# 0xSooki/stark-rs

Measured on AMD Instinct MI355X. Metric: ntt_field_elements_per_sec, higher is better.
Workload: dtype u32; 1 GPU; lde_2^22rows_x4cols_blowup8 (4 iNTT 2^22 + 4 coset NTT 2^25 per GPU per step); prime=469762049, parallelism=columns x1 (no collective)

## Files before the change

### stark_rs_amd/csrc/api.hip

```cpp
#include <condition_variable>
#include <functional>
#include <mutex>
#include <thread>

#include "hash_core.h"
#include "internal.h"
#include "lde_core.h"

const char *smi_status_string(int status) {
    switch (status) {
    case SMI_OK: return "ok";
    case SMI_ERR_NO_INVERSE: return "no inverse";
    case SMI_ERR_DIV_BY_ZERO: return "no division by zero";
    case SMI_ERR_POLY_DIV_BY_ZERO: return "No division by zero";
    case SMI_ERR_NOT_POW2: return "n must be a power of two";
    case SMI_ERR_ROOT_TOO_LARGE: return "n > 2^23 not supported by this modulus";
    case SMI_ERR_EMPTY_LEAVES: return "Cannot create tree from empty leaves";
    case SMI_ERR_LEAVES_NOT_POW2: return "Number of leaves must be power of 2";
    case SMI_ERR_INDEX_OOB: return "Index out of bounds";
    case SMI_ERR_DOMAIN_NOT_POW2: return "Domain length must be power of 2";
    case SMI_ERR_EXPANSION_NOT_POW2: return "Expansion factor must be power of 2";
    case SMI_ERR_EXPANSION_TOO_SMALL: return "Expansion factor must be at least 4";
    case SMI_ERR_CODEWORD_LEN: return "initial codeword length does not match domain length";
    case SMI_ERR_SAMPLE_ENTROPY: return "not enough entropy in indices wrt last codeword";
    case SMI_ERR_SAMPLE_TOO_MANY: return "cannot sample more indices than available in last codeword";
    case SMI_ERR_LEN_MISMATCH: return "assertion failed: domain.len() == values.len()";
    case SMI_ERR_EMPTY_DOMAIN: return "assertion failed: domain.len() > 0";
    case SMI_ERR_WRONG_FIELD: return "assertion failed: self.p == 998244353";
    case SMI_ERR_NO_ROUNDS: return "No FRI roots extracted";
    case SMI_ERR_BAD_ARG: return "bad argument";
    case SMI_ERR_NON_CANONICAL: return "field value not canonical (>= p)";
    case SMI_ERR_UNSUPPORTED_PRIME: return "unsupported modulus for this size";
    case SMI_ERR_NOT_GEOMETRIC: return "domain is not offset*omega^k";
    case SMI_ERR_COLUMNS_NOT_BOUND: return "proof has no column openings: it does not bind the column roots";
    case SMI_ERR_GRIND_EXHAUSTED: return "proof of work: no nonce below the search cap meets the difficulty";
    case SMI_ERR_HIP: return "HIP runtime error";
    case SMI_ERR_NO_DEVICE: return "no usable HIP device";
    case SMI_ERR_OOM: return "out of memory";
    case SMI_ERR_RCCL: return "RCCL / collective error";
    default: return "unknown status";
    }
}
const char *smi_version(void) { return "stark-mi 0.1 (gfx950)"; }
const char *smi_last_error(const smi_ctx *ctx) { return ctx ? ctx->err.c_str() : "null context"; }

int smi_fail(smi_ctx *ctx, int code, const char *msg) {
    if (ctx) ctx->err = msg ? msg : smi_status_string(code);
    return code;
}
int smi_hip_fail(smi_ctx *ctx, hipError_t e, const char *what) {
    if (ctx) ctx->err = std::string(what) + ": " + hipGetErrorString(e);
    (void)hipGetLastError();
    return e == hipErrorOutOfMemory ? SMI_ERR_OOM : SMI_ERR_HIP;
}

int smi_ctx_create(uint64_t p, uint64_t g, int device, smi_ctx **out) {
    if (!out) return SMI_ERR_BAD_ARG;
    *out = nullptr;
    int count = 0;
    if (hipGetDeviceCount(&count) != hipSuccess || count <= 0 || device < 0 || device >= count) return SMI_ERR_NO_DEVICE;
    smi_ctx *ctx = new smi_ctx();
    if (!field_setup(p, g, &ctx->fs)) {
        delete ctx;
        return SMI_ERR_UNSUPPORTED_PRIME;
    }
    ctx->device = device;
    int rc = SMI_OK;
    do {
        if (hipSetDevice(device) != hipSuccess) { rc = SMI_ERR_NO_DEVICE; break; }
        int cus = 0;
        if (hipDeviceGetAttribute(&cus, hipDeviceAttributeMultiprocessorCount, device) == hipSuccess && cus > 0) ctx->num_cus = cus;
        if (hipStreamCreateWithFlags(&ctx->stream, hipStreamNonBlocking) != hipSuccess) { rc = SMI_ERR_HIP; break; }
        ctx->own_stream = true;
        if (hipMalloc((void **)&ctx->d_flag, sizeof(int)) != hipSuccess) { rc = SMI_ERR_OOM; break; }
        if (hipMemsetAsync(ctx->d_flag, 0, sizeof(int), ctx->stream) != hipSuccess) { rc = SMI_ERR_HIP; break; }
        for (int dir = 0; dir < 2 && rc == SMI_OK; dir++) {
            GeomSpec sp[3];
            ntt_table_specs(ctx->fs, dir, sp);
            for (int k = 0; k < 3 && rc == SMI_OK; k++) {
                if (hipMalloc((void **)&ctx->d_tab[dir][k], ((size_t)sp[k].count * 4) << sp[k].pair) != hipSuccess) { rc = SMI_ERR_OOM; break; }
                rc = launch_geom_table(ctx, sp[k], ctx->d_tab[dir][k]);
            }
        }
        if (rc != SMI_OK) break;
        if (hipStreamSynchronize(ctx->stream) != hipSuccess) { rc = SMI_ERR_HIP; break; }
    } while (0);
    if (rc != SMI_OK) {
        smi_ctx_destroy(ctx);
        return rc;
    }
    *out = ctx;
    return SMI_OK;
}

void smi_ctx_destroy(smi_ctx *ctx) {
    if (!ctx) return;
    DeviceGuard dg__(ctx);
    (void)hipSetDevice(ctx->device);
    if (ctx->stream) (void)hipStreamSynchronize(ctx->stream);
    for (int d = 0; d < 2; d++)
        for (int k = 0; k < 3; k++) (void)hipFree(ctx->d_tab[d][k]);
    for (ScaleEntry &e : ctx->scale_cache) {
        (void)hipFree(e.lo);
        (void)hipFree(e.hi);
    }
    for (uint32_t *t : ctx->d_root_tab) (void)hipFree(t);
    (void)hipFree(ctx->scratch);
    (void)hipFree(ctx->arena);
    for (void *q : ctx->arena_overflow) (void)hipFree(q);
    for (int i = 0; i < 4; i++) (void)hipFree(ctx->tmp[i]);
    for (int i = 0; i < 2; i++) {
        if (ctx->pin[i]) (void)hipHostFree(ctx->pin[i]);
        if (ctx->pin_ev[i]) (void)hipEventDestroy(ctx->pin_ev[i]);
    }
    if (ctx->pin_out) (void)hipHostFree(ctx->pin_out);
    (void)hipFree(ctx->d_flag);
    if (ctx->own_stream && ctx->stream) (void)hipStreamDestroy(ctx->stream);
    delete ctx;
}

int smi_ctx_set_stream(smi_ctx *ctx, void *hip_stream) {
    if (!ctx) return SMI_ERR_BAD_ARG;
    DeviceGuard dg__(ctx);
    HIP_TRY(ctx, hipStreamSynchronize(ctx->stream));
    if (ctx->own_stream) (void)hipStreamDestroy(ctx->stream);
    ctx->stream = (hipStream_t)hip_stream;
    ctx->own_stream = false;
    return SMI_OK;
}
int smi_ctx_sync(smi_ctx *ctx) {
    if (!ctx) return SMI_ERR_BAD_ARG;
    DeviceGuard dg__(ctx);
    HIP_TRY(ctx, hipStreamSynchronize(ctx->stream));
    return SMI_OK;
}
int smi_ctx_profile(smi_ctx *ctx, int enable) {
    if (!ctx) return SMI_ERR_BAD_ARG;
    DeviceGuard dg__(ctx);
    ctx->prof_on = enable != 0;
    return SMI_OK;
}
int smi_ctx_profile_only(smi_ctx *ctx, const char *name_part) {
    if (!ctx) return SMI_ERR_BAD_ARG;
    if (name_part && strlen(name_part) >= sizeof ctx->prof_only) return smi_fail(ctx, SMI_ERR_BAD_ARG, "profile filter too long");
    memset(ctx->prof_only, 0, sizeof ctx->prof_only);
    if (name_part) memcpy(ctx->prof_only, name_part, strlen(name_part));
    return SMI_OK;
}
int smi_ctx_lde_two_pass(smi_ctx *ctx, int enable) {
    if (!ctx) return SMI_ERR_BAD_ARG;
    ctx->lde_two_pass = enable != 0;
    return SMI_OK;
}
int smi_ctx_copy_probe(smi_ctx *ctx, int enable) {
    if (!ctx) return SMI_ERR_BAD_ARG;
    DeviceGuard dg__(ctx);
    ctx->copy_probe = enable != 0;
    return SMI_OK;
}
int smi_ctx_profile_read(smi_ctx *ctx, smi_kernel_time *out, size_t cap, size_t *n) {
    if (!ctx || !n || (cap && !out)) return SMI_ERR_BAD_ARG;
    DeviceGuard dg__(ctx);
    HIP_TRY(ctx, hipStreamSynchronize(ctx->stream));
    size_t cnt = 0;
    for (ProfRec &r : ctx->prof) {
        float ms = 0.f;
        (void)hipEventElapsedTime(&ms, r.e0, r.e1);
        (void)hipEventDestroy(r.e0);
        (void)hipEventDestroy(r.e1);
        size_t k = 0;
        for (; k < cnt; k++)
            if (!strncmp(out[k].name, r.name, sizeof out[k].name - 1)) break;
        if (k == cnt) {
            if (cnt == cap) continue;
            memset(&out[k], 0, sizeof out[k]);
            strncpy(out[k].name, r.name, sizeof out[k].name - 1);
            cnt++;
        }
        out[k].launches++;
        out[k].total_ms += ms;
        out[k].alg_bytes += r.bytes;
        out[k].alg_mixes += r.mixes;
    }
    ctx->prof.clear();
    *n = cnt;
    return SMI_OK;
}
uint64_t smi_ctx_modulus(const smi_ctx *ctx) { return ctx ? ctx->fs.F.p : 0; }
uint32_t smi_ctx_two_adicity(const smi_ctx *ctx) { return ctx ? ctx->fs.K : 0; }

int ctx_pin_out(smi_ctx *ctx, size_t bytes, uint8_t **out) {
    if (bytes > ctx->pin_out_bytes) {
        HIP_TRY(ctx, hipStreamSynchronize(ctx->stream));
        if (ctx->pin_out) (void)hipHostFree(ctx->pin_out);
        ctx->pin_out = nullptr;
        ctx->pin_out_bytes = 0;
        const size_t want = bytes < ((size_t)2 << 20) ? ((size_t)2 << 20) : bytes + bytes / 4;
        if (hipHostMalloc(&ctx->pin_out, want, hipHostMallocDefault) != hipSuccess) {
            ctx->pin_out = nullptr;
            return smi_fail(ctx, SMI_ERR_OOM, "hipHostMalloc (result buffer)");
        }
        ctx->pin_out_bytes = want;
    }
    *out = (uint8_t *)ctx->pin_out;
    return SMI_OK;
}
int ctx_tmp(smi_ctx *ctx, int slot, size_t bytes, void **out) {
    if (bytes > ctx->tmp_bytes[slot]) {
        HIP_TRY(ctx, hipStreamSynchronize(ctx->stream));
        (void)hipFree(ctx->tmp[slot]);
        ctx->tmp[slot] = nullptr;
        ctx->tmp_bytes[slot] = 0;
        const size_t want = bytes + bytes / 4 + 256;
        if (hipMalloc(&ctx->tmp[slot], want) != hipSuccess) return smi_fail(ctx, SMI_ERR_OOM, "hipMalloc staging buffer");
        ctx->tmp_bytes[slot] = want;
    }
    *out = ctx->tmp[slot];
    return SMI_OK;
}
int arena_reset(smi_ctx *ctx) {
    if (!ctx->arena_overflow.empty() || ctx->arena_want > ctx->arena_size) {
        HIP_TRY(ctx, hipStreamSynchronize(ctx->stream));
        for (void *q : ctx->arena_overflow) (void)hipFree(q);
        ctx->arena_overflow.clear();
        if (ctx->arena_want > ctx->arena_size) {
            (void)hipFree(ctx->arena);
            ctx->arena = nullptr;
            ctx->arena_size = 0;
            const size_t want = ctx->arena_want + ctx->arena_want / 16 + (1u << 20);
            if (hipMalloc((void **)&ctx->arena, want) == hipSuccess) ctx->arena_size = want;
            else (void)hipGetLastError();
        }
    }
    ctx->arena_used = 0;
    ctx->arena_want = 0;
    return SMI_OK;
}
void *arena_alloc(smi_ctx *ctx, size_t bytes) {
    bytes = (bytes + 255) & ~(size_t)255;
    ctx->arena_want += bytes;
    if (ctx->arena_used + bytes <= ctx->arena_size) {
        void *q = ctx->arena + ctx->arena_used;
        ctx->arena_used += bytes;
        return q;
    }
    void *q = nullptr;
    if (hipMalloc(&q, bytes ? bytes : 256) != hipSuccess) {
        (void)hipGetLastError();
        return nullptr;
    }
    ctx->arena_overflow.push_back(q);
    return q;
}
int ctx_scratch(smi_ctx *ctx, size_t elems, uint32_t **out) {
    if (elems > ctx->scratch_elems) {
        HIP_TRY(ctx, hipStreamSynchronize(ctx->stream));
        (void)hipFree(ctx->scratch);
        ctx->scratch = nullptr;
        ctx->scratch_elems = 0;
        if (hipMalloc((void **)&ctx->scratch, elems * 4) != hipSuccess) return smi_fail(ctx, SMI_ERR_OOM, "hipMalloc NTT scratch");
        ctx->scratch_elems = elems;
    }
    *out = ctx->scratch;
    return SMI_OK;
}
NttTables ctx_tables(const smi_ctx *ctx, int inverse) {
    const int d = inverse ? 1 : 0;
    return NttTables{(const Tw2 *)ctx->d_tab[d][0], ctx->d_tab[d][1], ctx->d_tab[d][2], ctx->fs.K, ntt_table_h(ctx->fs.K)};
}
int ctx_root_table(smi_ctx *ctx, uint32_t log_m, const Tw2 **out) {
    if (log_m > 17 || log_m > ctx->fs.K) return smi_fail(ctx, SMI_ERR_BAD_ARG, "root table too large");
    if (!ctx->d_root_tab[log_m]) {
        const Fp &F = ctx->fs.F;
        const uint32_t w = h_root(ctx, log_m);
        const GeomSpec sp{F.r1, (uint32_t)(((uint64_t)w << 32) % F.p), 1, 1u << log_m, 1};
        uint32_t *d = nullptr;
        if (hipMalloc((void **)&d, ((size_t)8) << log_m) != hipSuccess) return smi_fail(ctx, SMI_ERR_OOM, "hipMalloc root table");
        const int rc = launch_geom_table(ctx, sp, d);
        if (rc != SMI_OK) {
            (void)hipFree(d);
            return rc;
        }
        ctx->d_root_tab[log_m] = d;
    }
    *out = (const Tw2 *)ctx->d_root_tab[log_m];
    return SMI_OK;
}
int ctx_scale_reserve(smi_ctx *ctx, size_t n) {
    if (ctx->scale_cache.size() + n < SMI_SCALE_CACHE_MAX) return SMI_OK;
    auto pinned = [&](const ScaleEntry &e) { return ctx->scale_depth > 0 && e.epoch == ctx->scale_epoch; };
    size_t want = ctx->scale_cache.size() / 2 > n ? ctx->scale_cache.size() / 2 : ctx->scale_cache.size();
    bool any = false;
    for (const ScaleEntry &e : ctx->scale_cache) any |= !pinned(e);
    if (!any) return SMI_OK;
    HIP_TRY(ctx, hipStreamSynchronize(ctx->stream));
    std::vector<ScaleEntry> keep;
    keep.reserve(ctx->scale_cache.size());
    for (const ScaleEntry &e : ctx->scale_cache) {
        if (want && !pinned(e)) {
            (void)hipFree(e.lo);
            (void)hipFree(e.hi);
            want--;
        } else {
            keep.push_back(e);
        }
    }
    ctx->scale_cache.swap(keep);
    return SMI_OK;
}
int ctx_scale_tables(smi_ctx *ctx, uint32_t c_plain, uint32_t q_plain, uint32_t L, ScaleTables *out) {
    for (ScaleEntry &e : ctx->scale_cache)
        if (e.c == c_plain && e.q == q_plain && e.L == L) {
            e.epoch = ctx->scale_epoch;
            *out = ScaleTables{e.lo, e.hi, scale_table_h(L)};
            return SMI_OK;
        }
    SMI_TRY(ctx_scale_reserve(ctx, 1));
    GeomSpec sp[2];
    scale_table_specs(ctx->fs.F, c_plain, q_plain, L, sp);
    ScaleEntry e{c_plain, q_plain, L, nullptr, nullptr, ctx->scale_epoch};
    if (hipMalloc((void **)&e.lo, (size_t)sp[0].count * 4) != hipSuccess) return smi_fail(ctx, SMI_ERR_OOM, "hipMalloc scale table");
    if (hipMalloc((void **)&e.hi, (size_t)sp[1].count * 4) != hipSuccess) {
        (void)hipFree(e.lo);
        return smi_fail(ctx, SMI_ERR_OOM, "hipMalloc scale table");
    }
    int rc = launch_geom_table(ctx, sp[0], e.lo);
    if (rc == SMI_OK) rc = launch_geom_table(ctx, sp[1], e.hi);
    if (rc != SMI_OK) {
        (void)hipFree(e.lo);
        (void)hipFree(e.hi);
        return rc;
    }
    ctx->scale_cache.push_back(e);
    *out = ScaleTables{e.lo, e.hi, scale_table_h(L)};
    return SMI_OK;
}
int check_flag(smi_ctx *ctx) {
    int flag = 0;
    HIP_TRY(ctx, hipMemcpyAsync(&flag, ctx->d_flag, sizeof(int), hipMemcpyDeviceToHost, ctx->stream));
    HIP_TRY(ctx, hipStreamSynchronize(ctx->stream));
    if (flag) {
        HIP_TRY(ctx, hipMemsetAsync(ctx->d_flag, 0, sizeof(int), ctx->stream));
        return smi_fail(ctx, SMI_ERR_NON_CANONICAL, "input field value >= p");
    }
    return SMI_OK;
}

static constexpr size_t SMI_PIN_CHUNK = (size_t)8 << 20;
static constexpr size_t SMI_PIN_MIN = (size_t)1 << 20;

static int ctx_pinned(smi_ctx *ctx) {
    for (int i = 0; i < 2; i++) {
        if (!ctx->pin[i] && hipHostMalloc(&ctx->pin[i], SMI_PIN_CHUNK * 4, hipHostMallocDefault) != hipSuccess) {
            ctx->pin[i] = nullptr;
            return smi_fail(ctx, SMI_ERR_OOM, "hipHostMalloc");
        }
        if (!ctx->pin_ev[i]) HIP_TRY(ctx, hipEventCreateWithFlags(&ctx->pin_ev[i], hipEventDisableTiming));
    }
    return SMI_OK;
}
namespace {
class HostPool {
    std::vector<std::thread> th_;
    std::mutex m_, run_m_;
    std::condition_variable work_, done_;
    std::function<void(size_t, size_t)> fn_;
    size_t n_ = 0, per_ = 0;
    unsigned gen_ = 0, pending_ = 0;
    bool stop_ = false;

    void worker(unsigned i) {
        unsigned seen = 0;
        for (;;) {
            std::unique_lock<std::mutex> lk(m_);
            work_.wait(lk, [&] { return stop_ || gen_ != seen; });
            if (stop_) return;
            seen = gen_;
            const size_t lo = (size_t)i * per_, hi = lo + per_ < n_ ? lo + per_ : n_;
            lk.unlock();
            if (lo < hi) fn_(lo, hi);
            lk.lock();
            if (--pending_ == 0) done_.notify_one();
        }
    }

public:
    explicit HostPool(unsigned t) {
        for (unsigned i = 1; i < t; i++) th_.emplace_back([this, i] { worker(i); });
    }
    ~HostPool() {
        {
            std::lock_guard<std::mutex> lk(m_);
            stop_ = true;
        }
        work_.notify_all();
        for (std::thread &x : th_) x.join();
    }
    unsigned size() const { return (unsigned)th_.size() + 1; }
    void run(size_t n, std::function<void(size_t, size_t)> fn) {
        std::lock_guard<std::mutex> serial(run_m_);
        const unsigned t = size();
        const size_t per = (n + t - 1) / t;
        {
            std::lock_guard<std::mutex> lk(m_);
            fn_ = fn;
            n_ = n;
            per_ = per;
            pending_ = t - 1;
            gen_++;
        }
        work_.notify_all();
        fn(0, per < n ? per : n);
        std::unique_lock<std::mutex> lk(m_);
        done_.wait(lk, [&] { return pending_ == 0; });
    }
};
}

template <class Fn> static void host_parallel(size_t n, Fn fn) {
    if (n < ((size_t)1 << 18)) {
        fn(0, n);
        return;
    }
    static HostPool pool([] {
        const char *e = getenv("SMI_HOST_THREADS");
        const int v = e ? atoi(e) : 0;
        unsigned hw = std::thread::hardware_concurrency();
        hw = hw < 1 ? 1 : hw;
        const unsigned cap = (unsigned)(v >= 1 && v <= 64 ? v : 8);
        return hw < cap ? hw : cap;
    }());
    pool.run(n, fn);
}

int dev_u32_to_host(smi_ctx *ctx, const uint32_t *d_in, size_t n, uint64_t *host) {
    if (!n) return SMI_OK;
    if (n < SMI_PIN_MIN) {
        void *stage;
        SMI_TRY(ctx_tmp(ctx, 0, n * 8, &stage));
        SMI_TRY(launch_widen(ctx, d_in, (uint64_t *)stage, n));
        HIP_TRY(ctx, hipMemcpyAsync(host, stage, n * 8, hipMemcpyDeviceToHost, ctx->stream));
        HIP_TRY(ctx, hipStreamSynchronize(ctx->stream));
        return SMI_OK;
    }
    SMI_TRY(ctx_pinned(ctx));
    const size_t nch = (n + SMI_PIN_CHUNK - 1) / SMI_PIN_CHUNK;
    for (size_t c = 0; c <= nch; c++) {
        if (c < nch) {
            const size_t off = c * SMI_PIN_CHUNK, cnt = n - off < SMI_PIN_CHUNK ? n - off : SMI_PIN_CHUNK;
            HIP_TRY(ctx, hipMemcpyAsync(ctx->pin[c & 1], d_in + off, cnt * 4, hipMemcpyDeviceToHost, ctx->stream));
            HIP_TRY(ctx, hipEventRecord(ctx->pin_ev[c & 1], ctx->stream));
        }
        if (c > 0) {
            const size_t off = (c - 1) * SMI_PIN_CHUNK, cnt = n - off < SMI_PIN_CHUNK ? n - off : SMI_PIN_CHUNK;
            HIP_TRY(ctx, hipEventSynchronize(ctx->pin_ev[(c - 1) & 1]));
            const uint32_t *src = (const uint32_t *)ctx->pin[(c - 1) & 1];
            uint64_t *dst = host + off;
            host_parallel(cnt, [=](size_t lo, size_t hi) {
                for (size_t i = lo; i < hi; i++) dst[i] = src[i];
            });
        }
    }
    return SMI_OK;
}

int host_to_dev_u32(smi_ctx *ctx, const uint64_t *host, size_t n, uint32_t *d_out, int reduce) {
    if (!n) return SMI_OK;
    if (n < SMI_PIN_MIN) {
        void *stage;
        SMI_TRY(ctx_tmp(ctx, 0, n * 8, &stage));
        HIP_TRY(ctx, hipMemcpyAsync(stage, host, n * 8, hipMemcpyHostToDevice, ctx->stream));
        SMI_TRY(launch_narrow(ctx, (const uint64_t *)stage, d_out, n, reduce));
        return check_flag(ctx);
    }
    SMI_TRY(ctx_pinned(ctx));
    const uint64_t p = ctx->fs.F.p;
    const size_t nch = (n + SMI_PIN_CHUNK - 1) / SMI_PIN_CHUNK;
    std::vector<int> bad(nch, 0);
    for (size_t c = 0; c < nch; c++) {
        const size_t off = c * SMI_PIN_CHUNK, cnt = n - off < SMI_PIN_CHUNK ? n - off : SMI_PIN_CHUNK;
        if (c >= 2) HIP_TRY(ctx, hipEventSynchronize(ctx->pin_ev[c & 1]));
        uint32_t *dst = (uint32_t *)ctx->pin[c & 1];
        const uint64_t *src = host + off;
        int *flag = &bad[c];
        host_parallel(cnt, [=](size_t lo, size_t hi) {
            uint64_t over = 0;
            if (reduce) {
                for (size_t i = lo; i < hi; i++) dst[i] = (uint32_t)(src[i] % p);
            } else {
                for (size_t i = lo; i < hi; i++) {
                    over |= (uint64_t)(src[i] >= p);
                    dst[i] = (uint32_t)src[i];
                }
            }
            if (over) __atomic_store_n(flag, 1, __ATOMIC_RELAXED);
        });
        HIP_TRY(ctx, hipMemcpyAsync(d_out + off, dst, cnt * 4, hipMemcpyHostToDevice, ctx->stream));
        HIP_TRY(ctx, hipEventRecord(ctx->pin_ev[c & 1], ctx->stream));
    }
    HIP_TRY(ctx, hipStreamSynchronize(ctx->stream));
    for (size_t c = 0; c < nch; c++)
        if (bad[c]) return smi_fail(ctx, SMI_ERR_NON_CANONICAL, "input field value >= p");
    return SMI_OK;
}


int smi_prim_nth_root(const smi_ctx *ctx, uint64_t n, uint64_t *out) {
    if (!ctx || !out) return SMI_ERR_BAD_ARG;
    if (!is_pow2(n)) return SMI_ERR_NOT_POW2;
    const uint32_t p = ctx->fs.F.p;
    if (ilog2(n) > ctx->fs.K) return p == 998244353u ? SMI_ERR_ROOT_TOO_LARGE : SMI_ERR_UNSUPPORTED_PRIME;
    *out = host_powmod(ctx->fs.g, (p - 1) / n, p);
    return SMI_OK;
}
int smi_ff_inv(const smi_ctx *ctx, uint64_t x, uint64_t *out) {
    if (!ctx || !out) return SMI_ERR_BAD_ARG;
    const uint32_t p = ctx->fs.F.p;
    if (x % p == 0) return SMI_ERR_NO_INVERSE;
    *out = h_inv(ctx, (uint32_t)(x % p));
    return SMI_OK;
}
int smi_ff_exp(const smi_ctx *ctx, uint64_t base, uint64_t e, uint64_t *out) {
    if (!ctx || !out) return SMI_ERR_BAD_ARG;
    *out = h_pow(ctx, (uint32_t)(base % ctx->fs.F.p), e);
    return SMI_OK;
}
int smi_ff_mul(const smi_ctx *ctx, uint64_t a, uint64_t b, uint64_t *out) {
    if (!ctx || !out) return SMI_ERR_BAD_ARG;
    const uint32_t p = ctx->fs.F.p;
    *out = h_mul(ctx, (uint32_t)(a % p), (uint32_t)(b % p));
    return SMI_OK;
}
int smi_domain_is_geometric(const smi_ctx *ctx, const uint64_t *domain, size_t n, uint64_t *offset) {
    if (!ctx || !domain || !n) return SMI_ERR_BAD_ARG;
    if (!is_pow2(n) || ilog2(n) > ctx->fs.K) return SMI_ERR_NOT_GEOMETRIC;
    const uint32_t p = ctx->fs.F.p, w = h_root(ctx, ilog2(n));
    if (domain[0] == 0 || domain[0] >= p) return SMI_ERR_NOT_GEOMETRIC;
    uint32_t x = (uint32_t)domain[0];
    for (size_t k = 1; k < n; k++) {
        x = host_mulmod(x, w, p);
        if (domain[k] != x) return SMI_ERR_NOT_GEOMETRIC;
    }
    if (offset) *offset = domain[0];
    return SMI_OK;
}

int smi_dev_alloc(smi_ctx *ctx, size_t bytes, void **d_ptr) {
    if (!ctx || !d_ptr) return SMI_ERR_BAD_ARG;
    DeviceGuard dg__(ctx);
    if (hipMalloc(d_ptr, bytes ? bytes : 1) != hipSuccess) return smi_fail(ctx, SMI_ERR_OOM, "hipMalloc");
    return SMI_OK;
}
int smi_dev_free(smi_ctx *ctx, void *d_ptr) {
    if (!ctx) return SMI_ERR_BAD_ARG;
    DeviceGuard dg__(ctx);
    HIP_TRY(ctx, hipStreamSynchronize(ctx->stream));
    HIP_TRY(ctx, hipFree(d_ptr));
    return SMI_OK;
}
int smi_dev_upload_u64(smi_ctx *ctx, const uint64_t *host, size_t n, uint32_t *d_out, int reduce) {
    if (!ctx || (!host && n) || (!d_out && n)) return SMI_ERR_BAD_ARG;
    DeviceGuard dg__(ctx);
    return host_to_dev_u32(ctx, host, n, d_out, reduce);
}
int smi_dev_download_u64(smi_ctx *ctx, const uint32_t *d_in, size_t n, uint64_t *host) {
    if (!ctx || (!host && n) || (!d_in && n)) return SMI_ERR_BAD_ARG;
    DeviceGuard dg__(ctx);
    return dev_u32_to_host(ctx, d_in, n, host);
}

int smi_dev_ntt(smi_ctx *ctx, const uint32_t *d_in, uint32_t *d_out, uint32_t log_n, size_t n_in, uint32_t batch,
// ... 437 lines not shown
```

### stark_rs_amd/csrc/emu.cpp

```cpp
#include <array>
#include <vector>

#include "ntt_driver.h"
#include "lde_core.h"
#include "tables.h"
#include "proof_parse.h"

namespace {

std::vector<uint32_t> fill(const GeomSpec &s, const Fp &F) {
    std::vector<uint32_t> t((size_t)s.count << s.pair);
    for (uint32_t i = 0; i < s.count; i++) {
        const uint32_t v = geom_entry(s.c_m, s.q_m, i, s.stride, F);
        if (s.pair) { const Tw2 c = tw2_from_mont(v, F); t[2 * i] = c.w; t[2 * i + 1] = c.q; }
        else t[i] = v;
    }
    return t;
}

template <int LOGR, int LOGW, int KIND, int CAP> void emu_pass_cols(const PassArgs &a) {
    typedef NttPass<LOGR, LOGW, KIND, CAP> NP;
    constexpr bool LAST = KIND == PASS_LAST;
    const uint32_t NT = NP::NT;
    std::vector<uint32_t> tile(NP::R * NP::WP);
    std::vector<Tw2> tw(NP::R);
    std::vector<std::array<uint32_t, 16>> mw(NT), mq(NT), iw(NT), regs(NT);
    const bool twin = KIND == PASS_MID && (a.flags & NTT_TW_IN);
    auto r16 = [](std::array<uint32_t, 16> &x) -> uint32_t(&)[16] { return reinterpret_cast<uint32_t(&)[16]>(x); };
    for (uint32_t blk = 0; blk < a.n_tiles; blk++) {
        typename NP::TileId t = NP::tile_id(a, blk);
        for (uint32_t tid = 0; tid < NT; tid++) NP::load_tw(a, tw.data(), tid);
        for (uint32_t b = 0; b < a.batch; b++) {
            if (b % NP::COLS_PER_WG == 0)
                for (uint32_t tid = 0; tid < NT; tid++) {
                    NP::out_mul(a, t, tid, r16(mw[tid]), r16(mq[tid]));
                    if (twin) NP::in_mul(a, t, tid, r16(iw[tid]));
                }
            if (twin) {
                for (uint32_t tid = 0; tid < NT; tid++) {
                    NP::template load_regs<0, false>(a, t, b, r16(regs[tid]), tid);
                    for (int i = 0; i < 16; i++) regs[tid][i] = mont_mul(regs[tid][i], iw[tid][i], a.F);
                }
                for (uint32_t tid = 0; tid < NT; tid++) NP::template step0_regs<0>(a, r16(regs[tid]), tile.data(), tw.data(), tid);
            } else if (!LAST) {
#define ZCASE(Z)                                                                                                 \
    case Z:                                                                                                      \
        for (uint32_t tid = 0; tid < NT; tid++) NP::template load_regs<Z>(a, t, b, r16(regs[tid]), tid);         \
        for (uint32_t tid = 0; tid < NT; tid++) NP::template step0_regs<Z>(a, r16(regs[tid]), tile.data(), tw.data(), tid); \
        break;
                switch (a.zlog) { ZCASE(2) ZCASE(3) ZCASE(4) default: ZCASE(0) }
#undef ZCASE
            } else if (a.flags & NTT_LAST_DIRECT) {
                for (uint32_t tid = 0; tid < NT; tid++) NP::load_rows_direct(a, t, b, r16(regs[tid]), tid);
                for (uint32_t tid = 0; tid < NT; tid++) NP::step0_rows(a, r16(regs[tid]), tile.data(), tw.data(), tid);
            } else {
                for (uint32_t tid = 0; tid < NT; tid++) NP::load_rows(a, t, b, r16(regs[tid]), tid);
                for (uint32_t tid = 0; tid < NT; tid++) NP::rows_to_lds(r16(regs[tid]), tile.data(), tid);
                for (uint32_t tid = 0; tid < NT; tid++) NP::step0_lds(a, tile.data(), tw.data(), tid);
            }
            for (uint32_t tid = 0; tid < NT; tid++) NP::step_mid(a, tile.data(), tw.data(), tid);
            for (uint32_t tid = 0; tid < NT; tid++) NP::last_step_store_mul(a, t, b, tile.data(), tw.data(), tid, r16(mw[tid]), r16(mq[tid]));
        }
    }
}

int g_share_cols = 1;

template <int LOGR, int LOGW, int KIND, int CAP> void emu_pass(const PassArgs &a, uint32_t batch) {
    typedef NttPass<LOGR, LOGW, KIND, CAP> NP;
    constexpr bool LAST = KIND == PASS_LAST;
    if (g_share_cols && NP::share_cols(a, g_share_cols == 2 ? 0u : (uint32_t)NP::COLS_MIN_WGS)) return emu_pass_cols<LOGR, LOGW, KIND, CAP>(a);
    std::vector<uint32_t> tile(NP::R * NP::WP);
    std::vector<Tw2> tw(NP::R);
    for (uint32_t b = 0; b < batch; b++)
        for (uint32_t blk = 0; blk < a.n_tiles; blk++) {
            typename NP::TileId t = NP::tile_id(a, blk);
            const uint32_t NT = NP::NT;
            for (uint32_t tid = 0; tid < NT; tid++) NP::load_tw(a, tw.data(), tid);
            if (!LAST) {
                std::vector<std::array<uint32_t, 16>> regs(NT);
#define ZCASE(Z)                                                                                                           \
    case Z:                                                                                                                \
        for (uint32_t tid = 0; tid < NT; tid++) NP::template load_regs<Z>(a, t, b, reinterpret_cast<uint32_t(&)[16]>(regs[tid]), tid); \
        for (uint32_t tid = 0; tid < NT; tid++) NP::template step0_regs<Z>(a, reinterpret_cast<uint32_t(&)[16]>(regs[tid]), tile.data(), tw.data(), tid); \
        break;
                switch (a.zlog) { ZCASE(0) ZCASE(1) ZCASE(2) ZCASE(3) ZCASE(4) }
#undef ZCASE
            } else if (a.flags & NTT_LAST_DIRECT) {
                std::vector<std::array<uint32_t, 16>> regs(NT);
                for (uint32_t tid = 0; tid < NT; tid++) NP::load_rows_direct(a, t, b, reinterpret_cast<uint32_t(&)[16]>(regs[tid]), tid);
                for (uint32_t tid = 0; tid < NT; tid++) NP::step0_rows(a, reinterpret_cast<uint32_t(&)[16]>(regs[tid]), tile.data(), tw.data(), tid);
            } else {
                for (uint32_t tid = 0; tid < NT; tid++) {
                    uint32_t v[16];
                    NP::load_rows(a, t, b, v, tid);
                    NP::rows_to_lds(v, tile.data(), tid);
                }
                for (uint32_t tid = 0; tid < NT; tid++) NP::step0_lds(a, tile.data(), tw.data(), tid);
            }
            for (uint32_t tid = 0; tid < NT; tid++) NP::step_mid(a, tile.data(), tw.data(), tid);
            for (uint32_t tid = 0; tid < NT; tid++) NP::last_step_store(a, t, b, tile.data(), tw.data(), tid);
        }
}

struct EmuLauncher {
    void small(const SmallArgs &a, uint32_t batch) {
        std::vector<uint32_t> buf((1u << a.L) + ((1u << a.L) >> 6) + 1);
        std::vector<Tw2> twm(((1u << a.L) >> 1) + 1);
        for (uint32_t tid = 0; tid < SMI_NTT_THREADS; tid++) NttSmall::load_tw(a, twm.data(), tid);
        for (uint32_t b = 0; b < batch; b++) {
            for (uint32_t tid = 0; tid < SMI_NTT_THREADS; tid++) NttSmall::load(a, b, buf.data(), tid);
            uint32_t s = 0;
            for (; s + 2 <= a.L; s += 2)
                for (uint32_t tid = 0; tid < SMI_NTT_THREADS; tid++) NttSmall::stage4(a, s, buf.data(), twm.data(), tid);
            if (s < a.L)
                for (uint32_t tid = 0; tid < SMI_NTT_THREADS; tid++) NttSmall::stage(a, s, buf.data(), twm.data(), tid);
            for (uint32_t tid = 0; tid < SMI_NTT_THREADS; tid++) NttSmall::store(a, b, buf.data(), tid);
        }
    }
    void pass(int logr, int logw, bool last, const PassArgs &a, uint32_t batch) {
#define X(LR, LW)                                           \
    if (logr == LR && logw == LW) {                         \
        const bool wide = a.F.p < (1u << 29);               \
        const int kind = last ? PASS_LAST : (a.flags & NTT_FIRST) ? PASS_FIRST : PASS_MID;   \
        if (wide && kind == PASS_FIRST) emu_pass<LR, LW, PASS_FIRST, 8>(a, batch);   \
        else if (wide && kind == PASS_MID) emu_pass<LR, LW, PASS_MID, 8>(a, batch);  \
        else if (wide) emu_pass<LR, LW, PASS_LAST, 8>(a, batch);                     \
        else if (kind == PASS_FIRST) emu_pass<LR, LW, PASS_FIRST, 4>(a, batch);      \
        else if (kind == PASS_MID) emu_pass<LR, LW, PASS_MID, 4>(a, batch);          \
        else emu_pass<LR, LW, PASS_LAST, 4>(a, batch);                               \
        return;                                             \
    }
        SMI_NTT_SHAPES(X)
#undef X
    }
};

}

static bool g_emu_last_direct = true;
extern "C" void emu_set_last_direct(int on) { g_emu_last_direct = on != 0; }
static int g_emu_defer_tw = 2;
extern "C" void emu_set_defer_tw(int mode) { g_emu_defer_tw = mode; }
extern "C" void emu_set_share_cols(int mode) { g_share_cols = mode; }
extern "C" int emu_ntt(uint64_t p, uint64_t g, const uint32_t *in, uint32_t *out, uint32_t L, uint32_t n_in,
                       uint32_t batch, uint64_t in_stride, uint64_t out_stride, int inverse, uint64_t offset,
                       uint64_t post_scale) {
    FieldSetup fs;
    if (!field_setup(p, g, &fs) || L > fs.K) return -1;
    const Fp &F = fs.F;
    GeomSpec sp[3];
    ntt_table_specs(fs, inverse, sp);
    std::vector<uint32_t> tw10 = fill(sp[0], F), lo = fill(sp[1], F), hi = fill(sp[2], F);
    NttRequest rq;
    memset(&rq, 0, sizeof rq);
    rq.T = NttTables{(const Tw2 *)tw10.data(), lo.data(), hi.data(), fs.K, ntt_table_h(fs.K)};
    std::vector<uint32_t> slo, shi;
    const uint32_t pp = F.p;
    if (!inverse) {
        rq.pre_scale = offset % pp != 1;
        if (rq.pre_scale) {
            GeomSpec s2[2];
            rq.q_plain = (uint32_t)(offset % pp);
            scale_table_specs(F, 1, (uint32_t)(offset % pp), L, s2);
            slo = fill(s2[0], F); shi = fill(s2[1], F);
        }
    } else {
        rq.post_scale = true;
        const uint32_t ninv = host_powmod((uint32_t)((1ull << L) % pp), pp - 2, pp);
        const uint32_t q = host_mulmod((uint32_t)(post_scale % pp), host_powmod((uint32_t)(offset % pp), pp - 2, pp), pp);
        GeomSpec s2[2];
        rq.q_plain = q;
        scale_table_specs(F, ninv, q, L, s2);
        slo = fill(s2[0], F); shi = fill(s2[1], F);
    }
    rq.S = ScaleTables{slo.data(), shi.data(), scale_table_h(L)};
    std::vector<uint32_t> scratch((size_t)batch << L);
    rq.in = in; rq.out = out; rq.scratch = scratch.data();
    rq.L = L; rq.n_in = n_in; rq.batch = batch; rq.in_stride = in_stride; rq.out_stride = out_stride; rq.F = F;
    rq.defer_tw = g_emu_defer_tw;
    rq.last_direct = g_emu_last_direct;
    EmuLauncher ln;
    return ntt_run(ln, rq) ? 0 : -1;
}

namespace {
struct EmuTables {
    std::vector<uint32_t> tw10, lo, hi, slo, shi;
    NttRequest rq;
};
bool emu_shard_request(uint64_t p, uint64_t g, uint32_t L, int inverse, uint64_t offset, EmuTables &t) {
    FieldSetup fs;
    if (!field_setup(p, g, &fs) || L > fs.K) return false;
    const Fp &F = fs.F;
    GeomSpec sp[3], s2[2];
    ntt_table_specs(fs, inverse, sp);
    t.tw10 = fill(sp[0], F); t.lo = fill(sp[1], F); t.hi = fill(sp[2], F);
    memset(&t.rq, 0, sizeof t.rq);
    t.rq.T = NttTables{(const Tw2 *)t.tw10.data(), t.lo.data(), t.hi.data(), fs.K, ntt_table_h(fs.K)};
    t.rq.L = L; t.rq.n_in = 1u << L; t.rq.batch = 1; t.rq.F = F;
    if (!inverse) {
        t.rq.pre_scale = offset % F.p != 1;
        t.rq.q_plain = (uint32_t)(offset % F.p);
        scale_table_specs(F, 1, t.rq.q_plain, L, s2);
    } else {
        t.rq.post_scale = true;
        t.rq.q_plain = 1;
        scale_table_specs(F, host_powmod((uint32_t)((1ull << L) % F.p), F.p - 2, F.p), 1, L, s2);
    }
    t.slo = fill(s2[0], F); t.shi = fill(s2[1], F);
    t.rq.S = ScaleTables{t.slo.data(), t.shi.data(), scale_table_h(L)};
    return true;
}
}
extern "C" int emu_ntt_shard_first(uint64_t p, uint64_t g, uint32_t *strip, uint32_t L, uint32_t log_g, uint32_t rank, int inverse, uint64_t offset) {
    EmuTables t;
    if (!emu_shard_request(p, g, L, inverse, offset, t)) return -1;
    t.rq.in = strip; t.rq.out = strip;
    EmuLauncher ln;
    return ntt_run_shard_first(ln, t.rq, log_g, rank) ? 0 : -1;
}
extern "C" int emu_ntt_shard_rest(uint64_t p, uint64_t g, uint32_t *rows, uint32_t *out, uint32_t L, uint32_t log_g, int inverse) {
    EmuTables t;
    if (!emu_shard_request(p, g, L, inverse, 1, t)) return -1;
    t.rq.scratch = rows; t.rq.out = out;
    t.rq.last_direct = g_emu_last_direct;
    EmuLauncher ln;
    return ntt_run_shard_rest(ln, t.rq, log_g) ? 0 : -1;
}

template <int LOGR, int CAP> void emu_lde_a(const LdeArgs &a) {
    typedef LdeA<LOGR, CAP> A;
    std::vector<uint32_t> tile(A::R * 4);
    std::vector<Tw2> tw(A::TWS);
    for (uint32_t b = 0; b < a.batch; b++)
        for (uint32_t blk = 0; blk < a.n_tiles; blk++) {
            const typename A::TileId t = A::tile_id(a, blk);
            std::vector<std::array<uint32_t, 16>> regs(A::NT);
            for (uint32_t tid = 0; tid < A::NT; tid++) A::load_tw(a, tw.data(), tid);
            for (uint32_t tid = 0; tid < A::NT; tid++) A::load_regs(a, t, b, reinterpret_cast<uint32_t(&)[16]>(regs[tid]), tid);
            for (uint32_t tid = 0; tid < A::NT; tid++) A::step0(a, reinterpret_cast<uint32_t(&)[16]>(regs[tid]), tile.data(), tw.data(), tid);
            for (uint32_t tid = 0; tid < A::NT; tid++) A::step_mid(a, tile.data(), tw.data(), tid);
            for (uint32_t tid = 0; tid < A::NT; tid++) A::last_step_store(a, t, b, tile.data(), tw.data(), tid);
        }
}
template <int CAP> void emu_lde_b(const LdeArgs &a) {
    typedef LdeB<CAP> B;
    std::vector<uint32_t> tile(B::R * B::WP);
    std::vector<Tw2> tw(B::R);
    for (uint32_t b = 0; b < a.batch; b++)
        for (uint32_t blk = 0; blk < a.n_tiles; blk++) {
            const typename B::TileId t = B::tile_id(a, blk);
            for (uint32_t tid = 0; tid < B::NT; tid++) B::load_tw(a, tw.data(), tid);
            for (uint32_t tid = 0; tid < B::NT; tid++) {
                uint32_t v[16];
                B::load(a, t, b, v, tid);
                B::to_lds(a, v, tile.data(), tid);
            }
            for (uint32_t tid = 0; tid < B::NT; tid++) B::step0(a, t, tile.data(), tw.data(), tid);
            for (uint32_t tid = 0; tid < B::NT; tid++) B::step_mid(a, tile.data(), tw.data(), tid);
            for (uint32_t tid = 0; tid < B::NT; tid++) B::last_step_store(a, t, b, tile.data(), tw.data(), tid);
        }
}
static int g_emu_lde_geo = -1, g_emu_lde_lay = -1;
extern "C" void emu_lde2_knobs(int geo_rq, int lay_kq) { g_emu_lde_geo = geo_rq; g_emu_lde_lay = lay_kq; }
extern "C" int emu_lde2(uint64_t p, uint64_t g, const uint32_t *coef, uint32_t *out, uint32_t L, uint32_t beta, uint32_t batch) {
    FieldSetup fs;
    if (!field_setup(p, g, &fs) || L + beta > fs.K || !lde2_supported(L, beta)) return -1;
    const Fp &F = fs.F;
    GeomSpec sp[3];
    ntt_table_specs(fs, 0, sp);
    std::vector<uint32_t> tw10 = fill(sp[0], F), lo = fill(sp[1], F), hi = fill(sp[2], F);
    std::vector<uint32_t> mid((size_t)batch << (L + beta)), coef_t((size_t)batch << L);
    const uint32_t log_m = L - SMI_LDE_LOGB + beta;
    const uint32_t wm = host_powmod(fs.wmax[0], 1ull << (fs.K - log_m), F.p);
    std::vector<uint32_t> ctab = fill(GeomSpec{F.r1, (uint32_t)(((uint64_t)wm << 32) % F.p), 1, 1u << log_m, 1}, F);
    LdeArgs a;
    memset(&a, 0, sizeof a);
    a.coef = coef; a.mid = mid.data(); a.coef_t = coef_t.data(); a.ctab = (const Tw2 *)ctab.data(); a.out = out; a.coef_stride = 1ull << L; a.out_stride = 1ull << (L + beta);
    a.F = F; a.T = NttTables{(const Tw2 *)tw10.data(), lo.data(), hi.data(), fs.K, ntt_table_h(fs.K)};
    a.L = L; a.beta = beta; a.batch = batch;
    a.geo_rq = g_emu_lde_geo >= 0 && (uint32_t)g_emu_lde_geo <= beta ? (uint32_t)g_emu_lde_geo : lde_default_geo_rq(beta);
    a.lay_kq = g_emu_lde_lay >= (int)(SMI_LDE_BLINES_LOG - a.geo_rq) && g_emu_lde_lay <= 4 ? (uint32_t)g_emu_lde_lay : SMI_LDE_BLINES_LOG - a.geo_rq;
    const bool wide = F.p < (1u << 29);
    const int logr = (int)L - SMI_LDE_LOGB;
    {
        std::vector<uint32_t> tile(LdeCoefTile::T * (LdeCoefTile::T + 1) * 4);
        for (uint32_t b = 0; b < batch; b++)
            for (uint32_t by = 0; by < (1u << logr) / LdeCoefTile::T; by++)
                for (uint32_t bx = 0; bx < 256 / LdeCoefTile::T; bx++) {
                    for (uint32_t tid = 0; tid < LdeCoefTile::NT; tid++) LdeCoefTile::load(a, bx, by, b, tile.data(), tid);
                    for (uint32_t tid = 0; tid < LdeCoefTile::NT; tid++) LdeCoefTile::store(a, bx, by, b, tile.data(), tid);
                }
    }
    a.n_tiles = 256u << beta;
#define LA(LR) if (logr == LR) { if (wide) emu_lde_a<LR, 8>(a); else emu_lde_a<LR, 4>(a); }
    LA(10) LA(11) LA(12)
#undef LA
    a.n_tiles = 1u << (L + beta - SMI_LDE_LOGB - SMI_LDE_BLINES_LOG);
    if (wide) emu_lde_b<8>(a); else emu_lde_b<4>(a);
    return 0;
}

#include "hash_core.h"
#include "merkle_plan.h"
extern "C" void emu_leaf_hash(const uint32_t *v, size_t n, uint8_t *out) {
    size_t i = 0;
    for (; i + 1 < n; i += 2) {
        uint32_t d0[8], d1[8];
        hashc::leaf_hash2(v[i], v[i + 1], d0, d1);
        memcpy(out + 32 * i, d0, 32);
        memcpy(out + 32 * (i + 1), d1, 32);
    }
    for (; i < n; i++) {
        uint32_t d[8];
        hashc::leaf_hash(v[i], d);
        memcpy(out + 32 * i, d, 32);
    }
}
extern "C" void emu_node_hash(const uint8_t *pairs, size_t n, uint8_t *out) {
    size_t i = 0;
    for (; i + 1 < n; i += 2) {
        uint32_t l0[8], r0[8], l1[8], r1[8], d0[8], d1[8];
        memcpy(l0, pairs + 64 * i, 32);
        memcpy(r0, pairs + 64 * i + 32, 32);
        memcpy(l1, pairs + 64 * (i + 1), 32);
        memcpy(r1, pairs + 64 * (i + 1) + 32, 32);
        hashc::node_hash2(l0, r0, l1, r1, d0, d1);
        memcpy(out + 32 * i, d0, 32);
        memcpy(out + 32 * (i + 1), d1, 32);
    }
    for (; i < n; i++) {
        uint32_t l[8], r[8], d[8];
        memcpy(l, pairs + 64 * i, 32);
        memcpy(r, pairs + 64 * i + 32, 32);
        hashc::node_hash(l, r, d);
        memcpy(out + 32 * i, d, 32);
    }
}
struct Q4 {
    uint32_t v[4];
    Q4() : v{0, 0, 0, 0} {}
    Q4(uint32_t x) : v{x, x, x, x} {}
    Q4(uint32_t a, uint32_t b, uint32_t c, uint32_t d) : v{a, b, c, d} {}
};
#define Q4_BIN(op)                                                 \
    inline Q4 operator op(const Q4 &a, const Q4 &b) {              \
        Q4 r;                                                      \
        for (int i = 0; i < 4; i++) r.v[i] = a.v[i] op b.v[i];     \
        return r;                                                  \
    }
Q4_BIN(+) Q4_BIN(^) Q4_BIN(&) Q4_BIN(|) Q4_BIN(*)
#undef Q4_BIN
inline Q4 operator<<(const Q4 &a, int sh) { return Q4(a.v[0] << sh, a.v[1] << sh, a.v[2] << sh, a.v[3] << sh); }
inline Q4 operator>>(const Q4 &a, int sh) { return Q4(a.v[0] >> sh, a.v[1] >> sh, a.v[2] >> sh, a.v[3] >> sh); }
namespace hashc {
#define Q4_MAP3(name)                                                          \
    inline Q4 name(const Q4 &a, const Q4 &b, const Q4 &c) {                    \
        Q4 r;                                                                  \
        for (int i = 0; i < 4; i++) r.v[i] = name(a.v[i], b.v[i], c.v[i]);     \
        return r;                                                              \
    }
Q4_MAP3(pk_mad_u16) Q4_MAP3(bfi32) Q4_MAP3(xor3) Q4_MAP3(add3)
#undef Q4_MAP3
inline Q4 dup_hi16(const Q4 &a) { return Q4(dup_hi16(a.v[0]), dup_hi16(a.v[1]), dup_hi16(a.v[2]), dup_hi16(a.v[3])); }
inline Q4 funnel16(const Q4 &hi, const Q4 &lo) {
    return Q4(funnel16(hi.v[0], lo.v[0]), funnel16(hi.v[1], lo.v[1]), funnel16(hi.v[2], lo.v[2]), funnel16(hi.v[3], lo.v[3]));
}
inline Q4 perm8(const Q4 &hi, const Q4 &lo, uint32_t sel) {
    return Q4(perm8(hi.v[0], lo.v[0], sel), perm8(hi.v[1], lo.v[1], sel), perm8(hi.v[2], lo.v[2], sel), perm8(hi.v[3], lo.v[3], sel));
}
inline void absorb32_words(Q4 P[8], const Q4 M[8]) {
    for (int i = 0; i < 4; i++) {
        uint32_t p[8], m[8];
        for (int j = 0; j < 8; j++) { p[j] = P[j].v[i]; m[j] = M[j].v[i]; }
        absorb32_words(p, m);
        for (int j = 0; j < 8; j++) P[j].v[i] = p[j];
    }
}
}
#define SMI_QUAD_EMU
namespace hashq {
#define SMI_QD inline
typedef Q4 word;
template <int P0, int P1, int P2, int P3> inline Q4 quad(const Q4 &x) { return Q4(x.v[P0], x.v[P1], x.v[P2], x.v[P3]); }
inline Q4 lane_in_quad(uint32_t) { return Q4(0, 1, 2, 3); }
inline Q4 mask_ge(const Q4 &q, uint32_t k) { return Q4(q.v[0] >= k ? ~0u : 0u, q.v[1] >= k ? ~0u : 0u, q.v[2] >= k ? ~0u : 0u, q.v[3] >= k ? ~0u : 0u); }
inline Q4 mask_eq(const Q4 &q, uint32_t k) { return Q4(q.v[0] == k ? ~0u : 0u, q.v[1] == k ? ~0u : 0u, q.v[2] == k ? ~0u : 0u, q.v[3] == k ? ~0u : 0u); }
inline Q4 sel4(const Q4 &q, const Q4 &a, const Q4 &b, const Q4 &c, const Q4 &d) {
    Q4 r;
    for (int i = 0; i < 4; i++) r.v[i] = q.v[i] == 0 ? a.v[i] : q.v[i] == 1 ? b.v[i] : q.v[i] == 2 ? c.v[i] : d.v[i];
    return r;
}
}
#include "hash_quad.h"
extern "C" void emu_node_hash_quad(const uint8_t *pairs, size_t n, uint8_t *out) {
    const hashq::Lane L = hashq::make_lane(0);
    for (size_t i = 0; i < n; i++) {
        uint32_t l[8], r[8], d[8];
        memcpy(l, pairs + 64 * i, 32);
        memcpy(r, pairs + 64 * i + 32, 32);
        Q4 ql[8], qr[8], lo, hi;
        for (int j = 0; j < 8; j++) { ql[j] = Q4(l[j]); qr[j] = Q4(r[j]); }
        hashq::node_hash(ql, qr, L, lo, hi);
        for (int q = 0; q < 4; q++) { d[q] = lo.v[q]; d[4 + q] = hi.v[q]; }
        memcpy(out + 32 * i, d, 32);
    }
}

struct H16 {
    uint32_t v[16];
    H16() { for (int i = 0; i < 16; i++) v[i] = 0; }
    H16(uint32_t x) { for (int i = 0; i < 16; i++) v[i] = x; }
};
#define H16_BIN(op)                                                \
    inline H16 operator op(const H16 &a, const H16 &b) {           \
        H16 r;                                                     \
        for (int i = 0; i < 16; i++) r.v[i] = a.v[i] op b.v[i];    \
        return r;                                                  \
    }
H16_BIN(+) H16_BIN(^) H16_BIN(&) H16_BIN(|) H16_BIN(*)
#undef H16_BIN
inline H16 operator<<(const H16 &a, int sh) { H16 r; for (int i = 0; i < 16; i++) r.v[i] = a.v[i] << sh; return r; }
inline H16 operator>>(const H16 &a, int sh) { H16 r; for (int i = 0; i < 16; i++) r.v[i] = a.v[i] >> sh; return r; }
namespace hashc {
#define H16_MAP3(name)                                                         \
    inline H16 name(const H16 &a, const H16 &b, const H16 &c) {                \
        H16 r;                                                                 \
        for (int i = 0; i < 16; i++) r.v[i] = name(a.v[i], b.v[i], c.v[i]);    \
        return r;                                                              \
    }
H16_MAP3(pk_mad_u16) H16_MAP3(bfi32) H16_MAP3(xor3)
#undef H16_MAP3
inline H16 funnel16(const H16 &hi, const H16 &lo) { H16 r; for (int i = 0; i < 16; i++) r.v[i] = funnel16(hi.v[i], lo.v[i]); return r; }
}
#define SMI_HEX_EMU
namespace hashx {
#define SMI_XD inline
typedef H16 word;
template <int N> inline H16 rot(const H16 &x) { H16 r; for (int i = 0; i < 16; i++) r.v[i] = x.v[(i - N) & 15]; return r; }
template <int N> inline H16 shr(const H16 &x) { H16 r; for (int i = 0; i < 16; i++) r.v[i] = i >= N ? x.v[i - N] : 0u; return r; }
template <int P0, int P1, int P2, int P3> inline H16 quad(const H16 &x) {
    const int P[4] = {P0, P1, P2, P3};
    H16 r;
    for (int i = 0; i < 16; i++) r.v[i] = x.v[(i & ~3) | P[i & 3]];
    return r;
}
inline H16 lane_in_row(uint32_t) { H16 r; for (int i = 0; i < 16; i++) r.v[i] = (uint32_t)i; return r; }
inline H16 mask_range(const H16 &w, uint32_t lo, uint32_t hi) { H16 r; for (int i = 0; i < 16; i++) r.v[i] = w.v[i] >= lo && w.v[i] < hi ? ~0u : 0u; return r; }
inline H16 table16(const H16 &w, const uint32_t (&t)[16]) { H16 r; for (int i = 0; i < 16; i++) r.v[i] = t[w.v[i] & 15]; return r; }
inline H16 perm8v(const H16 &hi, const H16 &lo, const H16 &sel) { H16 r; for (int i = 0; i < 16; i++) r.v[i] = hashc::perm8(hi.v[i], lo.v[i], sel.v[i]); return r; }
inline H16 lshl_or(const H16 &a, int sh, const H16 &b) { return (a << sh) | b; }
inline H16 lshl_add(const H16 &a, int sh, const H16 &b) { return (a << sh) + b; }
}
#include "hash_hex.h"
extern "C" void emu_node_hash_hex(const uint8_t *pairs, size_t n, uint8_t *out) {
    const hashx::Lane L = hashx::make_lane(0);
    for (size_t i = 0; i < n; i++) {
        uint32_t l[8], r[8];
        memcpy(l, pairs + 64 * i, 32);
        memcpy(r, pairs + 64 * i + 32, 32);
        H16 llo, lhi, rlo, rhi;
        for (int w = 0; w < 16; w++) { llo.v[w] = l[w >> 2]; lhi.v[w] = l[4 + (w >> 2)]; rlo.v[w] = r[w >> 2]; rhi.v[w] = r[4 + (w >> 2)]; }
        const H16 x = hashx::node_hash(hashx::message(llo, lhi, L), hashx::message(rlo, rhi, L), L);
        for (int w = 0; w < 16; w++) { out[32 * i + w] = (uint8_t)x.v[w]; out[32 * i + 16 + w] = (uint8_t)(x.v[w] >> 16); }
    }
}

extern "C" void emu_fs_round_hex(uint32_t *fs_words, const uint8_t *root, uint64_t *alpha) {
    const hashx::Lane L = hashx::make_lane(0);
    uint32_t r[8];
    memcpy(r, root, 32);
    H16 lo, hi, x;
    for (int w = 0; w < 16; w++) { lo.v[w] = r[w >> 2]; hi.v[w] = r[4 + (w >> 2)]; x.v[w] = fs_words[w]; }
    x = hashx::fs_absorb(x, hashx::message(lo, hi, L), L);
    for (int w = 0; w < 16; w++) fs_words[w] = x.v[w];
    const H16 y = hashx::fs_challenge(x, L);
    *alpha = 0;
    for (int k = 0; k < 8; k++) *alpha |= (uint64_t)(y.v[k] & 0xFFu) << (8 * k);
}
extern "C" void emu_fs_round(uint32_t *fs_words, const uint8_t *root, uint64_t *alpha) {
    uint32_t m[8];
    memcpy(m, root, 32);
    hashc::fs_absorb_root(fs_words, m, nullptr, alpha);
}
extern "C" void emu_fs_seed(const uint8_t *transcript, size_t len, uint32_t *fs_words, uint32_t *phase) {
    hashc::fs_seed(transcript, len, fs_words, phase);
}
extern "C" void emu_fs_absorb_root_phase(uint32_t *fs_words, uint32_t phase, const uint8_t *root, uint64_t *alpha) {
    uint32_t m[8];
    memcpy(m, root, 32);
    hashc::fs_absorb_root_phase(fs_words, m, phase, nullptr, alpha);
}
extern "C" uint64_t emu_fs_challenge_phase(const uint32_t *fs_words, uint32_t phase) { return hashc::fs_challenge_phase(fs_words, phase); }

extern "C" void emu_row_hash(const uint32_t *v, size_t n_rows, int W, uint8_t *out) {
    size_t i = 0;
    if (W >= 1 && W <= 4)
        for (; i + 1 < n_rows; i += 2) {
            uint32_t d0[8], d1[8];
            hashc::row_hash2(v + i * W, v + (i + 1) * W, W, d0, d1);
            memcpy(out + 32 * i, d0, 32);
            memcpy(out + 32 * (i + 1), d1, 32);
        }
    for (; i < n_rows; i++) {
        uint32_t d[8];
        hashc::row_hash(v + i * W, W, d);
        memcpy(out + 32 * i, d, 32);
    }
}
extern "C" void emu_row_hash_wide(const uint32_t *cols, size_t stride, size_t n, int W, uint8_t *out) {
    const uint32_t T = SMI_HASH_THREADS;
    const size_t blocks = ((n + 1) / 2 + T - 1) / T;
    for (size_t blk = 0; blk < blocks; blk++)
        for (uint32_t tid = 0; tid < T; tid++) {
            size_t i0, i1;
            bool two;
            if (!hashc::row_wide_pair(blk, tid, T, n, &i0, &i1, &two)) continue;
            uint32_t d0[8], d1[8];
            hashc::row_hash_wide2(cols, stride, i0, i1, W, d0, d1);
            memcpy(out + 32 * i0, d0, 32);
            if (two) memcpy(out + 32 * i1, d1, 32);
        }
}
extern "C" void emu_hash_bytes(const uint8_t *msg, size_t len, uint8_t *out) {
    uint32_t d[8];
    hashc::hash_bytes(msg, len, d);
    memcpy(out, d, 32);
}

#include "fri_core.h"
extern "C" int emu_fold_shard(uint64_t p, uint64_t g, const uint32_t *lo, const uint32_t *hi, uint32_t count, uint32_t i0,
                              uint32_t full_len, uint64_t alpha, uint64_t offset, uint64_t omega, uint32_t *out) {
    FieldSetup fs;
    if (!field_setup(p, g, &fs)) return -1;
    const Fp &F = fs.F;
    const uint32_t pp = F.p;
    uint32_t L = 0;
    while ((1u << L) < full_len / 2) L++;
    GeomSpec sp[2];
    scale_table_specs(F, host_powmod((uint32_t)offset, pp - 2, pp), host_powmod((uint32_t)omega, pp - 2, pp), L, sp);
    std::vector<uint32_t> slo = fill(sp[0], F), shi = fill(sp[1], F);
    const ScaleTables S{slo.data(), shi.data(), scale_table_h(L)};
    const uint32_t inv2_m = (uint32_t)(((uint64_t)host_powmod(2, pp - 2, pp) << 32) % pp);
    const uint32_t ah_m = fold_alpha_half(alpha, inv2_m, F);
    for (uint32_t i = 0; i < count; i++) out[i] = fold_element(lo[i], hi[i], i0 + i, ah_m, inv2_m, S, F);
    return 0;
}

extern "C" int emu_fold_ext(uint64_t p, uint64_t g, const uint32_t *in, uint32_t len, uint64_t stride, const uint64_t *alpha, uint64_t offset,
                            uint64_t omega, uint32_t *out, uint64_t out_stride) {
    FieldSetup fs;
    if (!field_setup(p, g, &fs) || !ext_field_ok(p, g, nullptr)) return -1;
    if (len < 2 || (len & (len - 1)) || stride < len || out_stride < len / 2 || !offset || !omega || offset >= p || omega >= p) return -1;
    const Fp &F = fs.F;
    const uint32_t pp = F.p, half = len / 2;
    uint32_t L = 0;
    while ((1u << L) < half) L++;
    GeomSpec sp[2];
    scale_table_specs(F, host_powmod((uint32_t)offset, pp - 2, pp), host_powmod((uint32_t)omega, pp - 2, pp), L, sp);
    std::vector<uint32_t> slo = fill(sp[0], F), shi = fill(sp[1], F);
    const ScaleTables S{slo.data(), shi.data(), scale_table_h(L)};
    const uint32_t inv2_m = (uint32_t)(((uint64_t)host_powmod(2, pp - 2, pp) << 32) % pp), g_m = (uint32_t)(((uint64_t)fs.g << 32) % pp);
    const ExtMul a = fold_ext_alpha(alpha, g_m, F);
    for (uint32_t i = 0; i < half; i++) {
        uint32_t l[4], h[4], o[4];
        for (int e = 0; e < 4; e++) {
            l[e] = in[e * stride + i];
            h[e] = in[e * stride + half + i];
        }
        fold_element_ext(l, h, i, a, inv2_m, S, F, o);
        for (int e = 0; e < 4; e++) out[e * out_stride + i] = o[e];
    }
    return 0;
}

extern "C" uint64_t emu_fs_rounds_ext(const uint8_t *prefix, size_t prefix_len, const uint8_t *roots, uint32_t n_roots, uint64_t *alphas) {
    uint32_t fs[16], phase = 0;
    hashc::fs_seed(prefix, prefix_len, fs, &phase);
    for (uint32_t r = 0; r < n_roots; r++) {
        uint32_t m[8];
        memcpy(m, roots + 32 * r, 32);
        if (r + 1 == n_roots) {
// ... 87 lines not shown
```

### stark_rs_amd/csrc/internal.h

```cpp
#pragma once
#include <string.h>
#include <hip/hip_runtime.h>

#include <stdlib.h>

#include <string>
#include <vector>

#include "../../include/stark_mi.h"
#include "fri_plan.h"
#include "tables.h"

struct ScaleEntry {
    uint32_t c, q, L;
    uint32_t *lo, *hi;
    uint64_t epoch;
};

struct ProfRec {
    const char *name;
    hipEvent_t e0, e1;
    double bytes;
    double mixes;
};

struct smi_ctx {
    int device = 0;
    int num_cus = 256;
    hipStream_t stream = nullptr;
    bool own_stream = false;
    FieldSetup fs;
    uint32_t *d_tab[2][3] = {{nullptr, nullptr, nullptr}, {nullptr, nullptr, nullptr}};
    std::vector<ScaleEntry> scale_cache;
    uint64_t scale_epoch = 1;
    int scale_depth = 0;
    uint32_t *d_root_tab[32] = {};
    uint32_t *scratch = nullptr;
    size_t scratch_elems = 0;
    void *tmp[4] = {nullptr, nullptr, nullptr, nullptr};
    size_t tmp_bytes[4] = {0, 0, 0, 0};
    int *d_flag = nullptr;
    void *pin[2] = {nullptr, nullptr};
    hipEvent_t pin_ev[2] = {nullptr, nullptr};
    void *pin_out = nullptr;
    size_t pin_out_bytes = 0;
    std::string err;
    bool prof_on = false;
    char prof_only[56] = {0};
    bool copy_probe = false;
    bool ntt_share_cols = !(getenv("SMI_NTT_SHARE_COLS") && atoi(getenv("SMI_NTT_SHARE_COLS")) == 0);
    bool ntt_twin_regs = !(getenv("SMI_NTT_TWIN_REGS") && atoi(getenv("SMI_NTT_TWIN_REGS")) == 0);
    bool ntt_last_direct = !(getenv("SMI_NTT_LAST_DIRECT") && atoi(getenv("SMI_NTT_LAST_DIRECT")) == 0);
    int ntt_defer_tw = getenv("SMI_NTT_DEFER_TW") ? (atoi(getenv("SMI_NTT_DEFER_TW")) != 0) : 2;
    bool lde_two_pass = getenv("SMI_LDE_TWO_PASS") && atoi(getenv("SMI_LDE_TWO_PASS"));
    std::vector<ProfRec> prof;
    uint8_t *arena = nullptr;
    size_t arena_size = 0, arena_used = 0, arena_want = 0;
    std::vector<void *> arena_overflow;
};
int arena_reset(smi_ctx *ctx);
void *arena_alloc(smi_ctx *ctx, size_t bytes);

struct ProfScope {
    smi_ctx *ctx;
    ProfRec r;
    bool on;
    ProfScope(smi_ctx *c, const char *name, double bytes, double mixes = 0.0) : ctx(c), on(c->prof_on) {
        if (on && c->prof_only[0] && !strstr(name, c->prof_only)) on = false;
        if (!on) return;
        r.name = name;
        r.bytes = bytes;
        r.mixes = mixes;
        if (hipEventCreate(&r.e0) != hipSuccess || hipEventCreate(&r.e1) != hipSuccess) { on = false; return; }
        (void)hipEventRecord(r.e0, ctx->stream);
    }
    ~ProfScope() {
        if (!on) return;
        (void)hipEventRecord(r.e1, ctx->stream);
        ctx->prof.push_back(r);
    }
};

struct DeviceGuard {
    int prev = -1;
    bool moved = false;
    explicit DeviceGuard(const smi_ctx *ctx) {
        if (!ctx) return;
        if (hipGetDevice(&prev) == hipSuccess && prev != ctx->device) moved = hipSetDevice(ctx->device) == hipSuccess;
    }
    ~DeviceGuard() {
        if (moved) (void)hipSetDevice(prev);
    }
};

struct smi_tree {
    smi_ctx *ctx;
    uint8_t *d_nodes;
    size_t n;
    bool owns;
};

int smi_hip_fail(smi_ctx *ctx, hipError_t e, const char *what);
#define HIP_TRY(ctx, call)                                             \
    do {                                                               \
        hipError_t e__ = (call);                                       \
        if (e__ != hipSuccess) return smi_hip_fail((ctx), e__, #call); \
    } while (0)
#define SMI_TRY(call)            \
    do {                         \
        int rc__ = (call);       \
        if (rc__ != SMI_OK) return rc__; \
    } while (0)

int smi_fail(smi_ctx *ctx, int code, const char *msg);
inline int smi_proof_out(smi_ctx *ctx, const std::vector<uint8_t> &bytes, uint8_t **proof, size_t *proof_len) {
    *proof = (uint8_t *)malloc(bytes.size() ? bytes.size() : 1);
    if (!*proof) return smi_fail(ctx, SMI_ERR_OOM, "malloc proof");
    memcpy(*proof, bytes.data(), bytes.size());
    *proof_len = bytes.size();
    return SMI_OK;
}

int ctx_tmp(smi_ctx *ctx, int slot, size_t bytes, void **out);
int ctx_scratch(smi_ctx *ctx, size_t elems, uint32_t **out);
int ctx_pin_out(smi_ctx *ctx, size_t bytes, uint8_t **out);
NttTables ctx_tables(const smi_ctx *ctx, int inverse);
int ctx_root_table(smi_ctx *ctx, uint32_t log_m, const Tw2 **out);
int ctx_scale_tables(smi_ctx *ctx, uint32_t c_plain, uint32_t q_plain, uint32_t L, ScaleTables *out);
#define SMI_SCALE_CACHE_MAX 96
int ctx_scale_reserve(smi_ctx *ctx, size_t n);
struct ScaleScope {
    smi_ctx *c;
    explicit ScaleScope(smi_ctx *ctx) : c(ctx) {
        if (c->scale_depth++ == 0) c->scale_epoch++;
    }
    ~ScaleScope() { c->scale_depth--; }
    ScaleScope(const ScaleScope &) = delete;
    ScaleScope &operator=(const ScaleScope &) = delete;
};

inline uint32_t h_mul(const smi_ctx *c, uint32_t a, uint32_t b) { return host_mulmod(a, b, c->fs.F.p); }
inline uint32_t h_pow(const smi_ctx *c, uint32_t a, uint64_t e) { return host_powmod(a, e, c->fs.F.p); }
inline uint32_t h_inv(const smi_ctx *c, uint32_t a) { return host_powmod(a, c->fs.F.p - 2, c->fs.F.p); }
inline uint32_t h_root(const smi_ctx *c, uint32_t log_n) {
    return host_powmod(c->fs.wmax[0], 1ull << (c->fs.K - log_n), c->fs.F.p);
}

struct FriTailRound {
    const uint32_t *cw;
    uint32_t *next;
    uint8_t *nodes;
    uint8_t *proof_slot;
    uint64_t *alpha_out;
    ScaleTables S;
    uint32_t len;
};
struct FriTailArgs {
    FriTailRound r[SMI_FRI_TAIL_MAX_ROUNDS];
    uint32_t n_rounds;
    uint32_t *fs_words;
    Fp F;
    uint32_t inv2_m;
    const uint32_t *pre_lo, *pre_hi;
    const uint64_t *pre_alpha;
    ScaleTables pre_S;
};
int launch_fri_tail(smi_ctx *ctx, const FriTailArgs &a);
uint64_t fri_tail_len();
struct FsSeed {
    uint32_t s[16];
    uint32_t phase;
};

enum { LEAF_LOAD = 0, LEAF_FOLD = 1, LEAF_COMBINE = 2 };
#define SMI_LEAF_COMBINE_MAX 8
struct LeafSrc {
    int kind;
    uint32_t *cw_out;
    Fp F;
    const uint32_t *lo, *hi;
    const uint64_t *alpha;
    ScaleTables S;
    uint32_t inv2_m;
    const uint32_t *cols;
    size_t stride;
    uint32_t n_cols;
    const uint32_t *weights_m;
};
struct FriRequest {
    const smi_fri_cfg *cfg;
    const uint32_t *d_codeword;
    size_t len;
    bool do_query;
    bool reset_arena = true;
    bool retain = false;
    const LeafSrc *round0_src = nullptr;
    const FsSeed *seed = nullptr;
    const void *ride_src = nullptr;
    size_t ride_bytes = 0;
    void *ride_dst = nullptr;
    FriRequest(const smi_fri_cfg *c, const uint32_t *cw, size_t n, bool query) : cfg(c), d_codeword(cw), len(n), do_query(query) {}
};
struct FriResult {
    FriLayout lay;
    std::vector<uint8_t> proof;
    std::vector<uint64_t> alphas;
    std::vector<uint64_t> top;
    smi_fri_run *run = nullptr;
};
int fri_run(smi_ctx *ctx, const FriRequest &rq, FriResult *res);

struct FriExtResult {
    std::vector<uint8_t> proof;
    std::vector<uint64_t> top;
    uint64_t nonce = 0;
};
#define SMI_GRIND_NONE (-1)
int fri_run_ext(smi_ctx *ctx, const smi_fri_cfg *cfg, const FsSeed *seed, const uint32_t *d_codeword, size_t len, size_t stride, bool reset_arena,
                FriExtResult *res, int grind = SMI_GRIND_NONE);
int grind_bits_check(smi_ctx *ctx, uint32_t bits);

int launch_leaf_hash(smi_ctx *ctx, const uint32_t *d_elems, size_t n, uint8_t *d_digests);
int launch_combine(smi_ctx *ctx, const uint8_t *d_in, size_t n_pairs, uint8_t *d_out);
int launch_hash_bytes(smi_ctx *ctx, const uint8_t *d_msg, size_t len, uint32_t *d_out);
int launch_hash_bytes_batch(smi_ctx *ctx, const uint8_t *d_msgs, size_t n, size_t len, uint32_t *d_out);
int launch_verify_paths(smi_ctx *ctx, const uint8_t *d_leaves, const uint64_t *d_idx, const uint8_t *d_paths, size_t k, uint32_t depth,
                        const uint8_t *d_root, uint8_t *d_ok);
int launch_merkle(smi_ctx *ctx, const uint32_t *d_elems, size_t n, uint8_t *d_nodes);
int launch_merkle_fs(smi_ctx *ctx, const uint32_t *d_elems, size_t n, uint8_t *d_nodes, uint32_t *fs_words, uint8_t *proof_slot,
                     uint64_t *alpha_out, bool *done);
int launch_merkle_src_fs(smi_ctx *ctx, const LeafSrc &src, size_t n, uint8_t *d_nodes, uint32_t *fs_words, uint8_t *proof_slot,
                         uint64_t *alpha_out, bool *done);
int launch_merkle_rows(smi_ctx *ctx, const uint32_t *d_cols, uint32_t n_cols, size_t col_stride, size_t n, uint8_t *d_nodes);
int launch_merkle_batch(smi_ctx *ctx, const uint32_t *d_elems, size_t n, uint8_t *d_nodes, uint32_t n_trees, size_t elem_stride,
                        size_t node_stride_bytes, uint32_t row_cols = 0, size_t row_stride = 0);
int launch_fold_shard(smi_ctx *ctx, const uint32_t *d_lo, const uint32_t *d_hi, size_t count, size_t i0, size_t full_len,
                      const uint64_t *d_alpha, uint64_t offset, uint64_t omega, uint32_t *d_out);
int fri_fold_tables(smi_ctx *ctx, uint32_t offset, uint32_t omega, uint64_t len, ScaleTables *S);
int ext_field_check(smi_ctx *ctx);
inline uint32_t fri_inv2_m(const smi_ctx *c) { return (uint32_t)(((uint64_t)h_inv(c, 2) << 32) % c->fs.F.p); }
int launch_fs_init(smi_ctx *ctx, void *fs, const FsSeed *seed);
int launch_fs_round(smi_ctx *ctx, void *fs, const uint8_t *root, uint8_t *proof_slot, uint64_t *alpha_out, uint32_t phase);
int launch_fs_challenge(smi_ctx *ctx, const void *fs, uint64_t *out, uint32_t phase);
int launch_sample_indices(smi_ctx *ctx, const uint64_t *challenge, uint64_t size, uint64_t reduced_size, uint32_t number,
                          uint64_t *indices, uint64_t *reduced);
int launch_emit_codeword(smi_ctx *ctx, const uint32_t *cw, uint64_t len, uint8_t *dst);
int launch_fs_weights(smi_ctx *ctx, const uint8_t *const *d_root_ptrs, uint32_t n, uint64_t *weights, uint8_t *roots_out);
int launch_geom_table(smi_ctx *ctx, const GeomSpec &s, uint32_t *d_out);
int launch_narrow(smi_ctx *ctx, const uint64_t *d_in, uint32_t *d_out, size_t n, int reduce);
int launch_widen(smi_ctx *ctx, const uint32_t *d_in, uint64_t *d_out, size_t n);
int dev_ntt(smi_ctx *ctx, const uint32_t *d_in, uint32_t *d_out, uint32_t log_n, size_t n_in, uint32_t batch,
            size_t in_stride, size_t out_stride, int inverse, uint64_t offset, uint64_t post_scale);
int dev_lde2(smi_ctx *ctx, const uint32_t *d_coef, uint32_t *d_out, uint32_t log_n, uint32_t log_blowup, uint32_t batch,
             size_t coef_stride, size_t out_stride);
int dev_ntt_shard_first(smi_ctx *ctx, uint32_t *d_strip, uint32_t log_n, uint32_t log_g, uint32_t rank, int inverse, uint64_t offset);
int dev_ntt_shard_rest(smi_ctx *ctx, uint32_t *d_rows, uint32_t *d_out, uint32_t log_n, uint32_t log_g, int inverse);
int dev_series_inv(smi_ctx *ctx, const uint32_t *rb, size_t k, uint32_t g0, uint32_t *g, uint32_t *e, uint32_t *f1, uint32_t *f2);
int check_flag(smi_ctx *ctx);
int host_to_dev_u32(smi_ctx *ctx, const uint64_t *host, size_t n, uint32_t *d_out, int reduce);
int dev_u32_to_host(smi_ctx *ctx, const uint32_t *d_in, size_t n, uint64_t *host);
struct AirHost;
int air_periodic_at(smi_ctx *ctx, const smi_stark_cfg *cfg, AirHost &H, const std::vector<uint64_t> &idx, std::vector<uint32_t> *out);
struct smi_air;
int air_host_tables(smi_ctx *ctx, const smi_stark_cfg *cfg, const smi_air *air, AirHost *H, uint64_t *E);
int air_compose_ext_launch(smi_ctx *ctx, AirHost &H, uint32_t *d_blob, const uint32_t *d_lde, size_t stride, const uint64_t *d_weights, uint32_t *d_out,
                           size_t out_stride);
int launch_air_row_open(smi_ctx *ctx, const uint32_t *d_cols, size_t stride, uint32_t W, const uint8_t *d_nodes, uint32_t depth, const uint64_t *d_top,
                        uint32_t t, uint32_t R, uint64_t B, uint8_t *d_out);
int air_periodic_tables(smi_ctx *ctx, const smi_stark_cfg *cfg, AirHost &H, uint32_t *d_vals, uint32_t *d_tab);
```

### stark_rs_amd/csrc/lde_core.h

```cpp
#pragma once
#include "ntt_core.h"

template <> struct Steps<12> { enum { n = 3, s0 = 4, s1 = 4, s2 = 4 }; };

#define SMI_LDE_LOGB 10
#define SMI_LDE_BLINES_LOG 4

struct LdeArgs {
    const uint32_t *coef;
    uint32_t *coef_t;
    uint32_t *mid;
    uint32_t *out;
    uint64_t coef_stride, out_stride;
    Fp F;
    NttTables T;
    const Tw2 *ctab;
    uint32_t L, beta;
    uint32_t n_tiles;
    uint32_t batch;
    uint32_t lay_kq;
    uint32_t geo_rq;
    uint32_t dbg;
};

SMI_HD uint32_t lde_kq_bits(uint32_t beta) { return SMI_LDE_BLINES_LOG - (beta < 2 ? beta : 2u); }

SMI_HD constexpr uint32_t lde_swz(uint32_t row) { return row ^ ((row >> 4) & 15u) ^ ((row >> 8) & 15u); }

struct LdeCoefTile {
    enum { T = 32, NT = 256 };
    static SMI_HD void load(const LdeArgs &a, uint32_t bx, uint32_t by, uint32_t batch, uint32_t *tile, uint32_t tid) {
        const uint32_t *col = a.coef + (uint64_t)batch * a.coef_stride;
#pragma unroll
        for (int i = 0; i < T * T / NT; i++) {
            const uint32_t e = tid + i * NT, row = e >> 5, c = e & 31u;
            const uint32_t j1 = by * T + row, jt = bx * T + c;
#pragma unroll
            for (int w = 0; w < 4; w++) tile[(row * (T + 1) + c) * 4 + w] = ld32(col, (j1 << SMI_LDE_LOGB) + (jt << 2) + w);
        }
    }
    static SMI_HD void store(const LdeArgs &a, uint32_t bx, uint32_t by, uint32_t batch, const uint32_t *tile, uint32_t tid) {
        uint32_t *dst = a.coef_t + ((uint64_t)batch << a.L);
        const uint32_t logR = a.L - SMI_LDE_LOGB;
#pragma unroll
        for (int i = 0; i < T * T / NT; i++) {
            const uint32_t e = tid + i * NT, c = e >> 5, row = e & 31u;
            const uint32_t j1 = by * T + row, jt = bx * T + c;
#pragma unroll
            for (int w = 0; w < 4; w++) st32(dst, (((jt << logR) + j1) << 2) + w, tile[(row * (T + 1) + c) * 4 + w]);
        }
    }
};

template <int LOGR, int CAP> struct LdeA {
    typedef Steps<LOGR> St;
    enum { R = 1 << LOGR, LOGW = 2, W = 4, TILE = R * W, NT = TILE / 16, V = 16, RL = 1 << St::s2, NB = 16 / RL };
    static_assert(St::n == 3 && St::s0 == 4, "three-step lines, radix-16 first step");

    struct TileId {
        uint32_t r;
        uint32_t jt;
    };
    static SMI_HD TileId tile_id(const LdeArgs &a, uint32_t block) {
        const uint32_t t = xcd_tile(block, a.n_tiles);
        TileId id;
        id.r = t & ((1u << a.beta) - 1u);
        id.jt = t >> a.beta;
        return id;
    }
    enum { TWS = R / 16 };
    static SMI_HD void load_tw(const LdeArgs &a, Tw2 *tws, uint32_t tid) {
        if (tid < (uint32_t)TWS) tws[tid] = a.T.tw10[tid << (SMI_TW_LOG + 4 - LOGR)];
    }
    static SMI_HD void load_regs(const LdeArgs &a, const TileId &t, uint32_t batch, uint32_t (&v)[V], uint32_t tid) {
        const uint32_t pos = tid >> 2;
        const uint32_t *col = a.coef_t + ((uint64_t)batch << a.L);
        const uint32_t o0 = (t.jt << (LOGR + 2)) + tid;
#pragma unroll
        for (int i = 0; i < V; i++) v[i] = ld32(col, o0 + (uint32_t)(i * (R / 4)));
        if (t.r) {
            const uint32_t mask = (1u << (LOGR + a.beta)) - 1u;
            const uint32_t e0 = t.r * pos, es = t.r * (uint32_t)(R / 16);
#pragma unroll
            for (int i = 0; i < V; i++) v[i] = shoup_mul(v[i], ld_tw(a.ctab, (e0 + (uint32_t)i * es) & mask), a.F.p);
        }
    }
    static SMI_HD void step0(const LdeArgs &a, uint32_t (&x)[V], uint32_t *tile, const Tw2 *tw, uint32_t tid) {
        const uint32_t w = tid & 3u, pos = tid >> 2, pos_sw = lde_swz(pos);
        int m[16];
#pragma unroll
        for (int i = 0; i < 16; i++) m[i] = 2;
        Tw2 t0[16];
#pragma unroll
        for (int kk = 1; kk < 16; kk++) t0[kk] = ld_tw(a.T.tw10, ((pos * kk) & (R - 1)) << (SMI_TW_LOG - LOGR));
        dft_regs<4, CAP>(x, m, tw, LOGR - 8, a.F);
#pragma unroll
        for (int kk = 0; kk < 16; kk++) {
            uint32_t v = x[brev<4>(kk)];
            int mv = m[brev<4>(kk)];
            if (kk) v = shoup_mul(v, t0[kk], a.F.p);
            else lz_fold_to2(v, mv, a.F.p);
            tile[((pos_sw ^ lde_swz((uint32_t)kk << (LOGR - 4))) << 2) + w] = v;
        }
    }
    static SMI_HD void step_mid(const LdeArgs &a, uint32_t *tile, const Tw2 *tw, uint32_t tid) {
        enum { S = St::s1, r = 1 << S, MLOG = LOGR - 4, SUB = MLOG - S, NBM = (TILE / r) / NT };
#pragma unroll
        for (int bi = 0; bi < NBM; bi++) {
            const uint32_t u = tid + bi * NT;
            const uint32_t w = u & 3u, ub = u >> 2;
            const uint32_t blk = ub >> SUB, pos = ub & ((1u << SUB) - 1u);
            const uint32_t base_sw = lde_swz((blk << MLOG) + pos);
            uint32_t x[r];
            int m[r];
#pragma unroll
            for (int q = 0; q < r; q++) {
                x[q] = tile[((base_sw ^ lde_swz((uint32_t)q << SUB)) << 2) + w];
                m[q] = 2;
            }
            dft_regs<S, CAP>(x, m, tw, MLOG - S, a.F);
#pragma unroll
            for (int kk = 0; kk < r; kk++) {
                uint32_t v = x[brev<S>(kk)];
                int mv = m[brev<S>(kk)];
                if (kk) v = shoup_mul(v, tw[(pos * kk) & (TWS - 1)], a.F.p);
                else lz_fold_to2(v, mv, a.F.p);
                tile[((base_sw ^ lde_swz((uint32_t)kk << SUB)) << 2) + w] = v;
            }
        }
    }
    static SMI_HD void last_step_store(const LdeArgs &a, const TileId &t, uint32_t batch, const uint32_t *tile, const Tw2 *tw,
                                       uint32_t tid) {
        enum { S1 = St::s1, SL = St::s2 };
        uint32_t *mid = a.mid + ((uint64_t)batch << (a.L + a.beta));
#pragma unroll
        for (int bi = 0; bi < NB; bi++) {
            const uint32_t u = tid + bi * NT;
            const uint32_t w = u & 3u, d0 = (u >> 2) & 15u, d1 = u >> 6;
            const uint32_t blk_sw = lde_swz(((d0 << S1) | d1) * RL);
            uint32_t x[RL];
            int m[RL];
#pragma unroll
            for (int q = 0; q < RL; q++) {
                x[q] = tile[((blk_sw ^ lde_swz((uint32_t)q)) << 2) + w];
                m[q] = 2;
            }
            dft_regs<SL, CAP>(x, m, tw, LOGR - 4 - SL, a.F);
            const uint32_t k1b = d0 | (d1 << 4);
            const uint32_t kq = a.lay_kq;
            const uint32_t o0 = ((((k1b >> kq) << a.beta) + t.r) << (10 + kq)) + (t.jt << (kq + 2)) + ((k1b & ((1u << kq) - 1u)) << 2) + w;
#pragma unroll
            for (int kk = 0; kk < RL; kk++) {
                const uint32_t val = lz_canon_m(x[brev<SL>(kk)], m[brev<SL>(kk)], a.F.p);
                if (!((a.dbg & 1u) && val != 0xFFFFFFFFu)) st32(mid, o0 + ((uint32_t)kk << (14 + S1 + a.beta)), val);
            }
        }
    }
};

template <int LOGR> struct LdeAProbe {
    typedef LdeA<LOGR, 4> A;
    static SMI_HD void run(const LdeArgs &a, uint32_t block, uint32_t batch, uint32_t tid) {
        typedef Steps<LOGR> St;
        const typename A::TileId t = A::tile_id(a, block);
        uint32_t v[16];
        LdeArgs b = a;
        const typename A::TileId t0 = {0u, t.jt};
        A::load_regs(b, t0, batch, v, tid);
        uint32_t *mid = a.mid + ((uint64_t)batch << (a.L + a.beta));
#pragma unroll
        for (int bi = 0; bi < A::NB; bi++) {
            const uint32_t u = tid + bi * A::NT;
            const uint32_t w = u & 3u, d0 = (u >> 2) & 15u, d1 = u >> 6, k1b = d0 | (d1 << 4);
            const uint32_t knob = (a.dbg >> 16) & 255u, kq = knob ? knob - 1u : a.lay_kq;
            const uint32_t o0 = ((((k1b >> kq) << a.beta) + t.r) << (10 + kq)) + (t.jt << (kq + 2)) + ((k1b & ((1u << kq) - 1u)) << 2) + w;
#pragma unroll
            for (int kk = 0; kk < A::RL; kk++) st32(mid, o0 + ((uint32_t)kk << (14 + St::s1 + a.beta)), v[bi * A::RL + kk] + 1u);
        }
    }
};

template <int CAP> struct LdeB {
    typedef NttPass<SMI_LDE_LOGB, SMI_LDE_BLINES_LOG, PASS_LAST, CAP> NP;
    enum { R = NP::R, W = NP::W, WP = NP::WP, NT = NP::NT, V = 16, RL = NP::RL, SL = NP::SL, NB = (NP::TILE / NP::RL) / NP::NT };

    struct Geo {
        uint32_t rq_bits, kq_bits, rh_bits;
    };
    static SMI_HD Geo geo(const LdeArgs &a) {
        Geo g;
        g.rq_bits = a.geo_rq;
        g.kq_bits = SMI_LDE_BLINES_LOG - g.rq_bits;
        g.rh_bits = a.beta - g.rq_bits;
        return g;
    }
    struct TileId {
        uint32_t k1_hi, rh;
    };
    static SMI_HD TileId tile_id(const LdeArgs &a, uint32_t block) {
        const Geo g = geo(a);
        const uint32_t t = xcd_tile(block, a.n_tiles);
        TileId id;
        id.rh = t & ((1u << g.rh_bits) - 1u);
        id.k1_hi = t >> g.rh_bits;
        return id;
    }
    static SMI_HD void load_tw(const LdeArgs &a, Tw2 *tw, uint32_t tid) {
        PassArgs pa;
        pa.T = a.T;
        NP::load_tw(pa, tw, tid);
    }
    static SMI_HD uint32_t in_addr(const LdeArgs &a, const Geo &g, const TileId &t, uint32_t e) {
        const uint32_t rq = e >> (10 + g.kq_bits), jt = (e >> (g.kq_bits + 2)) & 255u, k1q = (e >> 2) & ((1u << g.kq_bits) - 1u), j0lo = e & 3u;
        const uint32_t k1 = (t.k1_hi << g.kq_bits) | k1q, r = (t.rh << g.rq_bits) | rq;
        return ((((k1 >> a.lay_kq) << a.beta) + r) << (10 + a.lay_kq)) + (jt << (a.lay_kq + 2)) + ((k1 & ((1u << a.lay_kq) - 1u)) << 2) + j0lo;
    }
    static SMI_HD void load(const LdeArgs &a, const TileId &t, uint32_t batch, uint32_t (&v)[V], uint32_t tid) {
        static_assert(NT == 1024 && V == 16, "thread / load-index split of the tile's 14 element bits");
        const Geo g = geo(a);
        const uint32_t *mid = a.mid + ((uint64_t)batch << (a.L + a.beta));
        const uint32_t base = in_addr(a, g, t, tid);
        const uint32_t jt_stride = (256u >> g.kq_bits) << (a.lay_kq + 2), r_stride = 1u << (10 + a.lay_kq), imask = (1u << g.kq_bits) - 1u;
#pragma unroll
        for (int i = 0; i < V; i++) v[i] = ld32(mid, base + ((uint32_t)i & imask) * jt_stride + ((uint32_t)i >> g.kq_bits) * r_stride);
    }
    static SMI_HD void to_lds(const LdeArgs &a, const uint32_t (&v)[V], uint32_t *tile, uint32_t tid) {
        const Geo g = geo(a);
        const uint32_t k1q = (tid >> 2) & ((1u << g.kq_bits) - 1u), j0lo = tid & 3u, jt_lo = tid >> (g.kq_bits + 2);
        const uint32_t base = ((jt_lo << 2) + j0lo) * WP + k1q;
        const uint32_t jt_stride = (256u >> g.kq_bits) * 4u * WP, r_stride = 1u << g.kq_bits, imask = (1u << g.kq_bits) - 1u;
#pragma unroll
        for (int i = 0; i < V; i++) tile[base + ((uint32_t)i & imask) * jt_stride + ((uint32_t)i >> g.kq_bits) * r_stride] = v[i];
    }
    static SMI_HD void step0(const LdeArgs &a, const TileId &t, uint32_t *tile, const Tw2 *tw, uint32_t tid) {
        const Geo g = geo(a);
        const uint32_t l = tid & (W - 1), pos = tid >> SMI_LDE_BLINES_LOG;
        const uint32_t r = (t.rh << g.rq_bits) | (l >> g.kq_bits), k1 = (t.k1_hi << g.kq_bits) | (l & ((1u << g.kq_bits) - 1u));
        const uint32_t E = r + (k1 << a.beta), sh = a.T.K - (a.L + a.beta);
        uint32_t cur = two_level(a.T.lo, a.T.hi, a.T.h, (pos * E) << sh, a.F);
        const uint32_t ratio = two_level(a.T.lo, a.T.hi, a.T.h, (E << 6) << sh, a.F), rq = ratio * a.F.pinv;
        uint32_t x[16];
        int m[16];
#pragma unroll
        for (int q = 0; q < 16; q++) {
            x[q] = mont_mul(tile[(pos + ((uint32_t)q << 6)) * WP + l], cur, a.F);
            m[q] = 1;
            if (q + 1 < 16) cur = mont_mul_c(cur, ratio, rq, a.F);
        }
        dft_regs<4, CAP>(x, m, tw, SMI_LDE_LOGB - 4, a.F);
#pragma unroll
        for (int kk = 0; kk < 16; kk++) {
            uint32_t v = x[brev<4>(kk)];
            int mv = m[brev<4>(kk)];
            if (kk) v = shoup_mul(v, tw[(pos * kk) & (R - 1)], a.F.p);
            else lz_fold_to2(v, mv, a.F.p);
            tile[(pos + ((uint32_t)kk << 6)) * WP + l] = v;
        }
    }
    static SMI_HD void step_mid(const LdeArgs &a, uint32_t *tile, const Tw2 *tw, uint32_t tid) {
        PassArgs pa;
        pa.F = a.F;
        NP::step_mid(pa, tile, tw, tid);
    }
    static SMI_HD void last_step_store(const LdeArgs &a, const TileId &t, uint32_t batch, const uint32_t *tile, const Tw2 *tw,
                                       uint32_t tid) {
        const Geo g = geo(a);
        uint32_t *out = a.out + (uint64_t)batch * a.out_stride;
        const uint32_t logRA = a.L - SMI_LDE_LOGB, ksh = a.beta + logRA;
        const uint32_t base = ((t.k1_hi << g.kq_bits) << a.beta) + (t.rh << g.rq_bits);
#pragma unroll
        for (int bi = 0; bi < NB; bi++) {
            const uint32_t u = tid + bi * NT;
            const uint32_t l = u & (W - 1), blk = u >> SMI_LDE_BLINES_LOG;
            uint32_t x[RL];
            int m[RL];
#pragma unroll
            for (int q = 0; q < RL; q++) {
                x[q] = tile[(blk * RL + q) * WP + l];
                m[q] = 2;
            }
            dft_regs<SL, CAP>(x, m, tw, SMI_LDE_LOGB - SL, a.F);
            const uint32_t k0b = NP::blk_to_k(blk);
            const uint32_t lineoff = ((l & ((1u << g.kq_bits) - 1u)) << a.beta) + (l >> g.kq_bits);
            const uint32_t o0 = (k0b << ksh) + base + lineoff;
#pragma unroll
            for (int kk = 0; kk < RL; kk++) {
                const uint32_t val = lz_canon_m(x[brev<SL>(kk)], m[brev<SL>(kk)], a.F.p);
                if (!((a.dbg & 2u) && val != 0xFFFFFFFFu)) st32(out, o0 + ((uint32_t)kk << (SMI_LDE_LOGB - SL + ksh)), val);
            }
        }
    }
};

struct LdeBProbe {
    typedef LdeB<4> B;
    static SMI_HD void run(const LdeArgs &a, uint32_t block, uint32_t batch, uint32_t tid) {
        const uint32_t var = (a.dbg >> 8) & 255u;
        B::Geo g = B::geo(a);
        if (var == 1 && a.beta >= 3) { g.rq_bits = 3; g.kq_bits = 1; g.rh_bits = a.beta - 3; }
        if (var == 2) { g.rq_bits = 1; g.kq_bits = 3; g.rh_bits = a.beta - 1; }
        const uint32_t *mid = a.mid + ((uint64_t)batch << (a.L + a.beta));
        uint32_t *out = a.out + (uint64_t)batch * a.out_stride;
        const uint32_t ksh = a.beta + a.L - SMI_LDE_LOGB;
        const uint32_t reps = var == 3 ? 2u : 1u;
        for (uint32_t rep = 0; rep < reps; rep++) {
            uint32_t t = var == 4 ? block : xcd_tile(block, a.n_tiles);
            if (var == 3) t = 2u * xcd_tile(block, a.n_tiles / 2u) + rep;
            B::TileId id;
            id.rh = t & ((1u << g.rh_bits) - 1u);
            id.k1_hi = t >> g.rh_bits;
            uint32_t v[16];
#pragma unroll
            for (int i = 0; i < 16; i++) v[i] = ld32(mid, B::in_addr(a, g, id, (uint32_t)(i * B::NT) + tid));
            const uint32_t base = ((id.k1_hi << g.kq_bits) << a.beta) + (id.rh << g.rq_bits);
            if (var == 5) {
                const uint32_t l = tid & 15u, row0 = tid >> 4;
                const uint32_t line0 = ((id.k1_hi << g.kq_bits) << a.beta) & ~31u;
#pragma unroll
                for (int i = 0; i < 8; i++) {
                    const uint32_t k0 = row0 + (uint32_t)i * 64u + ((id.rh & 1u) << 9);
                    st32(out, (k0 << ksh) + line0 + 2u * l, v[2 * i] + 1u);
                    st32(out, (k0 << ksh) + line0 + 2u * l + 1u, v[2 * i + 1] + 1u);
                }
                continue;
            }
#pragma unroll
            for (int bi = 0; bi < B::NB; bi++) {
                const uint32_t u = tid + bi * B::NT;
                const uint32_t l = u & (B::W - 1), blk = u >> SMI_LDE_BLINES_LOG;
                const uint32_t lineoff = ((l & ((1u << g.kq_bits) - 1u)) << a.beta) + (l >> g.kq_bits);
                const uint32_t o0 = (B::NP::blk_to_k(blk) << ksh) + base + lineoff;
#pragma unroll
                for (int kk = 0; kk < B::RL; kk++) st32(out, o0 + ((uint32_t)kk << (SMI_LDE_LOGB - B::SL + ksh)), v[bi * B::RL + kk] + 1u);
            }
        }
    }
};

SMI_HD uint32_t lde_default_geo_rq(uint32_t beta) { return beta < 2 ? beta : 2u; }
inline bool lde2_supported(uint32_t L, uint32_t beta) { return L >= 20 && L <= 22 && beta >= 1 && beta <= 4; }
```

### stark_rs_amd/csrc/ntt.hip

```cpp
#include "internal.h"
#include "ntt_driver.h"
#include "lde_core.h"

template <int LOGR, int LOGW, int KIND, int CAP>
__global__ __launch_bounds__(1 << (LOGR + LOGW - 4)) void ntt_pass_kernel(const PassArgs a) {
    typedef NttPass<LOGR, LOGW, KIND, CAP> NP;
    __shared__ uint32_t tile[NP::R * NP::WP];
    __shared__ Tw2 tw[NP::R];
    const uint32_t tid = threadIdx.x, batch = blockIdx.y;
    const typename NP::TileId t = NP::tile_id(a, blockIdx.x);
    NP::load_tw(a, tw, tid);
    uint32_t v[NP::V];
    if constexpr (KIND == PASS_FIRST) {
#define ZCASE(Z)                                         \
    case Z:                                              \
        NP::template load_regs<Z>(a, t, batch, v, tid);  \
        __syncthreads();       \
        NP::template step0_regs<Z>(a, v, tile, tw, tid); \
        break;
        switch (a.zlog) { ZCASE(2) ZCASE(3) ZCASE(4) default: ZCASE(0) }
#undef ZCASE
    } else if constexpr (KIND == PASS_MID) {
        NP::template load_regs<0>(a, t, batch, v, tid);
        __syncthreads();
        NP::template step0_regs<0>(a, v, tile, tw, tid);
    } else if (a.flags & NTT_LAST_DIRECT) {
        NP::load_rows_direct(a, t, batch, v, tid);
        __syncthreads();
        NP::step0_rows(a, v, tile, tw, tid);
    } else {
        NP::load_rows(a, t, batch, v, tid);
        NP::rows_to_lds(v, tile, tid);
        __syncthreads();
        NP::step0_lds(a, tile, tw, tid);
    }
    __syncthreads();
    if (NP::St::n == 3) {
        NP::step_mid(a, tile, tw, tid);
        __syncthreads();
    }
    NP::last_step_store(a, t, batch, tile, tw, tid);
}

#ifndef SMI_COLS_WAVES
#define SMI_COLS_WAVES(TILE_LOG, LOGR) ((TILE_LOG) >= 14 || (LOGR) >= 11 ? 4 : ((LOGR) == 10 ? 5 : 6))
#endif
#ifndef SMI_COLS_TWIN_WAVES
#define SMI_COLS_TWIN_WAVES 4
#endif
#ifndef SMI_COLS_TWIN_MQ
#define SMI_COLS_TWIN_MQ 1
#endif
#ifndef SMI_COLS_PREFETCH
#define SMI_COLS_PREFETCH 1
#endif
template <int LOGR, int LOGW, int KIND, int CAP, bool TWIN = false>
__global__ __launch_bounds__(1 << (LOGR + LOGW - 4), TWIN ? SMI_COLS_TWIN_WAVES : SMI_COLS_WAVES(LOGR + LOGW, LOGR)) void ntt_pass_cols_kernel(const PassArgs a) {
    typedef NttPass<LOGR, LOGW, KIND, CAP> NP;
    __shared__ uint32_t tile[NP::R * NP::WP];
    __shared__ Tw2 tw[NP::R];
    const uint32_t tid0 = threadIdx.x;
    const typename NP::TileId t = NP::tile_id(a, blockIdx.x);
    NP::load_tw(a, tw, tid0);
    constexpr bool MQ = !TWIN || SMI_COLS_TWIN_MQ;
    uint32_t mw[NP::V], mq[MQ ? NP::V : 1];
    NP::template out_mul<MQ>(a, t, tid0, mw, mq);
    uint32_t iw[TWIN ? NP::V : 1];
    if constexpr (TWIN) NP::in_mul(a, t, tid0, iw);
    const uint32_t col0 = blockIdx.y * NP::COLS_PER_WG, col1 = min(a.batch, col0 + (uint32_t)NP::COLS_PER_WG);
    if constexpr (SMI_COLS_PREFETCH && KIND == PASS_MID && LOGW == 5) {
        uint32_t v[NP::V];
        auto load = [&](uint32_t col) {
            uint32_t tid = tid0;
            asm volatile("" : "+v"(tid));
            NP::template load_regs<0, !TWIN>(a, t, col, v, tid);
        };
        load(col0);
        for (uint32_t batch = col0; batch < col1; batch++) {
            uint32_t tid = tid0;
            asm volatile("" : "+v"(tid));
            if constexpr (TWIN) {
#pragma unroll
                for (int i = 0; i < NP::V; i++) v[i] = mont_mul(v[i], iw[i], a.F);
            }
            __syncthreads();
            NP::template step0_regs<0>(a, v, tile, tw, tid);
            if (batch + 1 < col1) load(batch + 1);
            __syncthreads();
            if (NP::St::n == 3) {
                NP::step_mid(a, tile, tw, tid);
                __syncthreads();
            }
            NP::template last_step_store_mul<MQ>(a, t, batch, tile, tw, tid, mw, mq);
        }
        return;
    }
    for (uint32_t batch = col0; batch < col1; batch++) {
        uint32_t tid = tid0;
        asm volatile("" : "+v"(tid));
        uint32_t v[NP::V];
        static_assert(KIND != PASS_FIRST, "first passes keep one workgroup per (tile, column), NttPass::share_cols");
        if constexpr (KIND == PASS_MID) {
            NP::template load_regs<0, !TWIN>(a, t, batch, v, tid);
            if constexpr (TWIN) {
#pragma unroll
                for (int i = 0; i < NP::V; i++) v[i] = mont_mul(v[i], iw[i], a.F);
            }
            __syncthreads();
            NP::template step0_regs<0>(a, v, tile, tw, tid);
        } else if (a.flags & NTT_LAST_DIRECT) {
            NP::load_rows_direct(a, t, batch, v, tid);
            __syncthreads();
            NP::step0_rows(a, v, tile, tw, tid);
        } else {
            NP::load_rows(a, t, batch, v, tid);
            if (batch != col0) __syncthreads();
            NP::rows_to_lds(v, tile, tid);
            __syncthreads();
            NP::step0_lds(a, tile, tw, tid);
        }
        __syncthreads();
        if (NP::St::n == 3) {
            NP::step_mid(a, tile, tw, tid);
            __syncthreads();
        }
        NP::template last_step_store_mul<MQ>(a, t, batch, tile, tw, tid, mw, mq);
    }
}

template <int LOGR, int LOGW, int KIND>
__global__ __launch_bounds__(1 << (LOGR + LOGW - 4)) void ntt_copy_probe_kernel(const PassArgs a) {
    typedef NttPass<LOGR, LOGW, KIND, 4> NP;
    enum { NB = (NP::TILE / NP::RL) / NP::NT, KSTEP_LOG = LOGR - NP::SL };
    const uint32_t tid = threadIdx.x, batch = blockIdx.y;
    const typename NP::TileId t = NP::tile_id(a, blockIdx.x);
    uint32_t v[NP::V];
    const uint32_t lin = a.flags >> 30;
    const uint64_t lin_in = (uint64_t)batch * a.in_stride + (uint64_t)blockIdx.x * NP::TILE;
    const uint64_t lin_out = (uint64_t)batch * a.out_stride + (uint64_t)blockIdx.x * NP::TILE;
    if ((lin & 1u) && KIND != PASS_FIRST) {
#pragma unroll
        for (int i = 0; i < NP::V; i++) v[i] = ld32(a.in + lin_in, (uint32_t)i * NP::NT + tid);
    } else if constexpr (KIND == PASS_LAST) {
        if (a.flags & NTT_LAST_DIRECT) NP::load_rows_direct(a, t, batch, v, tid);
        else NP::load_rows(a, t, batch, v, tid);
    } else if constexpr (KIND == PASS_MID) {
        NP::template load_regs<0, false>(a, t, batch, v, tid);
    } else {
        switch (a.zlog) {
        case 2: NP::template load_regs<2>(a, t, batch, v, tid); break;
        case 3: NP::template load_regs<3>(a, t, batch, v, tid); break;
        case 4: NP::template load_regs<4>(a, t, batch, v, tid); break;
        default: NP::template load_regs<0>(a, t, batch, v, tid); break;
        }
    }
    if ((lin & 2u) && KIND != PASS_LAST) {
#pragma unroll
        for (int i = 0; i < NP::V; i++) st32(a.out + lin_out, (uint32_t)i * NP::NT + tid, v[i] + 1u);
        return;
    }
    uint32_t *out = a.out + (uint64_t)batch * a.out_stride + t.out_base;
    const uint32_t sh = KIND == PASS_LAST ? a.Sp : a.L - a.Sp - LOGR;
#pragma unroll
    for (int bi = 0; bi < NB; bi++) {
        const uint32_t u = tid + bi * NP::NT;
        const uint32_t o0 = (NP::blk_to_k(u >> LOGW) << sh) + (u & (NP::W - 1));
#pragma unroll
        for (int kk = 0; kk < NP::RL; kk++) st32(out, o0 + ((uint32_t)kk << (KSTEP_LOG + sh)), v[bi * NP::RL + kk] + 1u);
    }
}

__global__ __launch_bounds__(256) void lde_coef_tile_kernel(const LdeArgs a) {
    __shared__ uint32_t tile[LdeCoefTile::T * (LdeCoefTile::T + 1) * 4];
    LdeCoefTile::load(a, blockIdx.x, blockIdx.y, blockIdx.z, tile, threadIdx.x);
    __syncthreads();
    LdeCoefTile::store(a, blockIdx.x, blockIdx.y, blockIdx.z, tile, threadIdx.x);
}
template <int LOGR, int CAP>
__global__ __launch_bounds__(1 << (LOGR - 2)) void lde_a_kernel(const LdeArgs a) {
    typedef LdeA<LOGR, CAP> A;
    __shared__ uint32_t tile[A::R * 4];
    __shared__ Tw2 tw[A::TWS];
    const uint32_t tid = threadIdx.x, batch = blockIdx.y;
    const typename A::TileId t = A::tile_id(a, blockIdx.x);
    A::load_tw(a, tw, tid);
    uint32_t v[A::V];
    A::load_regs(a, t, batch, v, tid);
    __syncthreads();
    A::step0(a, v, tile, tw, tid);
    __syncthreads();
    A::step_mid(a, tile, tw, tid);
    __syncthreads();
    A::last_step_store(a, t, batch, tile, tw, tid);
}
template <int CAP>
__global__ __launch_bounds__(1024) void lde_b_kernel(const LdeArgs a) {
    typedef LdeB<CAP> B;
    __shared__ uint32_t tile[B::R * B::WP];
    __shared__ Tw2 tw[B::R];
    const uint32_t tid = threadIdx.x, batch = blockIdx.y;
    const typename B::TileId t = B::tile_id(a, blockIdx.x);
    B::load_tw(a, tw, tid);
    uint32_t v[B::V];
    B::load(a, t, batch, v, tid);
    B::to_lds(a, v, tile, tid);
    __syncthreads();
    B::step0(a, t, tile, tw, tid);
    __syncthreads();
    B::step_mid(a, tile, tw, tid);
    __syncthreads();
    B::last_step_store(a, t, batch, tile, tw, tid);
}

template <int LOGR> __global__ __launch_bounds__(1 << (LOGR - 2)) void lde_a_probe_kernel(const LdeArgs a) {
    LdeAProbe<LOGR>::run(a, blockIdx.x, blockIdx.y, threadIdx.x);
}
__global__ __launch_bounds__(1024) void lde_b_probe_kernel(const LdeArgs a) { LdeBProbe::run(a, blockIdx.x, blockIdx.y, threadIdx.x); }

__global__ __launch_bounds__(SMI_NTT_THREADS) void ntt_small_kernel(const SmallArgs a) {
    __shared__ uint32_t buf[SMI_TILE + SMI_TILE / 64];
    __shared__ Tw2 twm[SMI_TILE / 2];
    const uint32_t tid = threadIdx.x, batch = blockIdx.x;
    NttSmall::load_tw(a, twm, tid);
    NttSmall::load(a, batch, buf, tid);
    __syncthreads();
    uint32_t s = 0;
    for (; s + 2 <= a.L; s += 2) {
        NttSmall::stage4(a, s, buf, twm, tid);
        __syncthreads();
    }
    if (s < a.L) {
        NttSmall::stage(a, s, buf, twm, tid);
        __syncthreads();
    }
    NttSmall::store(a, batch, buf, tid);
}

__global__ void geom_table_kernel(uint32_t *out, GeomSpec s, Fp F) {
    const uint32_t i = blockIdx.x * blockDim.x + threadIdx.x;
    if (i >= s.count) return;
    const uint32_t v = geom_entry(s.c_m, s.q_m, i, s.stride, F);
    if (s.pair) {
        const Tw2 c = tw2_from_mont(v, F);
        out[2 * i] = c.w;
        out[2 * i + 1] = c.q;
    } else {
        out[i] = v;
    }
}

__global__ void narrow_kernel(const uint64_t *in, uint32_t *out, size_t n, uint32_t p, int reduce, int *flag) {
    size_t i = (size_t)blockIdx.x * blockDim.x + threadIdx.x;
    const size_t step = (size_t)gridDim.x * blockDim.x;
    int bad = 0;
    for (; i < n; i += step) {
        const uint64_t v = in[i];
        if (v >= p) bad = 1;
        out[i] = (uint32_t)(v % p);
    }
    if (bad && !reduce) *flag = 1;
}
__global__ void widen_kernel(const uint32_t *in, uint64_t *out, size_t n) {
    size_t i = (size_t)blockIdx.x * blockDim.x + threadIdx.x;
    const size_t step = (size_t)gridDim.x * blockDim.x;
    for (; i < n; i += step) out[i] = in[i];
}

static uint32_t grid_for(size_t n, uint32_t block) {
    size_t g = (n + block - 1) / block;
    return (uint32_t)(g > 2048 ? 2048 : (g ? g : 1));
}

int launch_geom_table(smi_ctx *ctx, const GeomSpec &s, uint32_t *d_out) {
    geom_table_kernel<<<(s.count + 255) / 256, 256, 0, ctx->stream>>>(d_out, s, ctx->fs.F);
    HIP_TRY(ctx, hipGetLastError());
    return SMI_OK;
}
int launch_narrow(smi_ctx *ctx, const uint64_t *d_in, uint32_t *d_out, size_t n, int reduce) {
    if (!n) return SMI_OK;
    narrow_kernel<<<grid_for(n, 256), 256, 0, ctx->stream>>>(d_in, d_out, n, ctx->fs.F.p, reduce, ctx->d_flag);
    HIP_TRY(ctx, hipGetLastError());
    return SMI_OK;
}
int launch_widen(smi_ctx *ctx, const uint32_t *d_in, uint64_t *d_out, size_t n) {
    if (!n) return SMI_OK;
    widen_kernel<<<grid_for(n, 256), 256, 0, ctx->stream>>>(d_in, d_out, n);
    HIP_TRY(ctx, hipGetLastError());
    return SMI_OK;
}

namespace {
struct HipLauncher {
    smi_ctx *ctx;
    hipError_t err = hipSuccess;
    void small(const SmallArgs &a, uint32_t batch) {
        ProfScope ps(ctx, "ntt_small_kernel", (4.0 * a.n_in + 4.0 * (1ull << a.L)) * batch);
        ntt_small_kernel<<<batch, SMI_NTT_THREADS, 0, ctx->stream>>>(a);
        note();
    }
    template <int LR, int LW, int KIND, int CAP> void launch(const PassArgs &a) {
        if constexpr (KIND != PASS_FIRST) {
            if (ctx->ntt_share_cols && NttPass<LR, LW, KIND, CAP>::share_cols(a)) {
                const dim3 grid(a.n_tiles, NttPass<LR, LW, KIND, CAP>::col_groups(a));
                if (KIND == PASS_MID && (a.flags & NTT_TW_IN) && ctx->ntt_twin_regs)
                    ntt_pass_cols_kernel<LR, LW, KIND, CAP, KIND == PASS_MID><<<grid, 1 << (LR + LW - 4), 0, ctx->stream>>>(a);
                else
                    ntt_pass_cols_kernel<LR, LW, KIND, CAP><<<grid, 1 << (LR + LW - 4), 0, ctx->stream>>>(a);
                return;
            }
        }
        ntt_pass_kernel<LR, LW, KIND, CAP><<<dim3(a.n_tiles, a.batch), 1 << (LR + LW - 4), 0, ctx->stream>>>(a);
    }
    template <int LR, int LW> void launch_probe(int kind, const PassArgs &a0) {
        static const uint32_t lin = getenv("SMI_PROBE_LINEAR") ? (uint32_t)atoi(getenv("SMI_PROBE_LINEAR")) & 3u : 0u;
        PassArgs a = a0;
        a.flags |= lin << 30;
        const dim3 grid(a.n_tiles, a.batch);
        if (kind == PASS_FIRST) ntt_copy_probe_kernel<LR, LW, PASS_FIRST><<<grid, 1 << (LR + LW - 4), 0, ctx->stream>>>(a);
        else if (kind == PASS_MID) ntt_copy_probe_kernel<LR, LW, PASS_MID><<<grid, 1 << (LR + LW - 4), 0, ctx->stream>>>(a);
        else ntt_copy_probe_kernel<LR, LW, PASS_LAST><<<grid, 1 << (LR + LW - 4), 0, ctx->stream>>>(a);
    }
    template <int LR, int LW, int CAP> void launch_kind(int kind, const PassArgs &a) {
        if (kind == PASS_FIRST) launch<LR, LW, PASS_FIRST, CAP>(a);
        else if (kind == PASS_MID) launch<LR, LW, PASS_MID, CAP>(a);
        else launch<LR, LW, PASS_LAST, CAP>(a);
    }
    void pass(int logr, int logw, bool last, const PassArgs &a, uint32_t batch) {
        const double n = (double)(1ull << (a.L - a.shard_log));
        const double bytes = ((a.flags & NTT_FIRST) && !a.shard_log ? 4.0 * a.n_in : 4.0 * n) * batch + 4.0 * n * batch;
        const bool wide = a.F.p < (1u << 29);
        const int kind = last ? PASS_LAST : (a.flags & NTT_FIRST) ? PASS_FIRST : PASS_MID;
#define X(LR, LW)                                                                                              \
    if (logr == LR && logw == LW) {                                                                            \
        if (ctx->copy_probe) {                                                                                 \
            ProfScope ps(ctx, kind == PASS_LAST ? "ntt_copy_probe<" #LR "," #LW ",last>" : kind == PASS_MID ? "ntt_copy_probe<" #LR "," #LW ",mid>" : "ntt_copy_probe<" #LR "," #LW ",first>", bytes); \
            launch_probe<LR, LW>(kind, a);                                                                     \
            note();                                                                                            \
            return;                                                                                            \
        }                                                                                                      \
        const bool cols = ctx->ntt_share_cols && (kind == PASS_LAST ? NttPass<LR, LW, PASS_LAST, 4>::share_cols(a)                     \
                                                  : kind == PASS_MID ? NttPass<LR, LW, PASS_MID, 4>::share_cols(a) : false);            \
        ProfScope ps(ctx, cols ? (kind == PASS_LAST ? "ntt_pass_cols_kernel<" #LR "," #LW ",last>" : "ntt_pass_cols_kernel<" #LR "," #LW ",mid>") \
                          : kind == PASS_LAST ? "ntt_pass_kernel<" #LR "," #LW ",last>" : kind == PASS_MID ? "ntt_pass_kernel<" #LR "," #LW ",mid>" : "ntt_pass_kernel<" #LR "," #LW ",first>", bytes); \
        if (wide) launch_kind<LR, LW, 8>(kind, a);                                                             \
        else launch_kind<LR, LW, 4>(kind, a);                                                                  \
        note();                                                                                                \
        return;                                                                                                \
    }
        SMI_NTT_SHAPES(X)
#undef X
        if (err == hipSuccess) err = hipErrorInvalidValue;
    }
    void note() {
        hipError_t e = hipGetLastError();
        if (err == hipSuccess) err = e;
    }
};
}

int dev_lde2(smi_ctx *ctx, const uint32_t *d_coef, uint32_t *d_out, uint32_t log_n, uint32_t log_blowup, uint32_t batch,
             size_t coef_stride, size_t out_stride) {
    if (!lde2_supported(log_n, log_blowup) || log_n + log_blowup > ctx->fs.K) return smi_fail(ctx, SMI_ERR_BAD_ARG, "lde2: unsupported shape");
    if (!batch) return SMI_OK;
    if (batch > 65535) return smi_fail(ctx, SMI_ERR_BAD_ARG, "batch too large");
    const uint32_t logN = log_n + log_blowup;
    LdeArgs a;
    memset(&a, 0, sizeof a);
    a.coef = d_coef; a.out = d_out; a.coef_stride = coef_stride; a.out_stride = out_stride;
    a.F = ctx->fs.F; a.T = ctx_tables(ctx, 0); a.L = log_n; a.beta = log_blowup; a.batch = batch;
    SMI_TRY(ctx_root_table(ctx, log_n - SMI_LDE_LOGB + log_blowup, &a.ctab));
    SMI_TRY(ctx_scratch(ctx, ((size_t)batch << logN) + ((size_t)batch << log_n), &a.mid));
    a.coef_t = a.mid + ((size_t)batch << logN);
    const bool wide = a.F.p < (1u << 29);
    const double n = (double)(1ull << log_n), N = (double)(1ull << logN);
    static const uint32_t dbg = getenv("SMI_LDE_DBG") ? (uint32_t)atoi(getenv("SMI_LDE_DBG")) : 0u;
    static const int env_geo = getenv("SMI_LDE_GEO") ? atoi(getenv("SMI_LDE_GEO")) : -1, env_lay = getenv("SMI_LDE_LAYOUT") ? atoi(getenv("SMI_LDE_LAYOUT")) : -1;
    a.dbg = dbg;
    a.geo_rq = env_geo >= 0 && (uint32_t)env_geo <= log_blowup && env_geo <= 4 ? (uint32_t)env_geo : lde_default_geo_rq(log_blowup);
    a.lay_kq = env_lay >= (int)(SMI_LDE_BLINES_LOG - a.geo_rq) && env_lay <= 4 ? (uint32_t)env_lay : SMI_LDE_BLINES_LOG - a.geo_rq;
    const int logr = (int)log_n - SMI_LDE_LOGB;
    {
        ProfScope ps(ctx, "lde_coef_tile_kernel", 8.0 * n * batch);
        lde_coef_tile_kernel<<<dim3(256 / LdeCoefTile::T, (1u << logr) / LdeCoefTile::T, batch), LdeCoefTile::NT, 0, ctx->stream>>>(a);
        HIP_TRY(ctx, hipGetLastError());
    }
    if (ctx->copy_probe) {
        a.n_tiles = 256u << log_blowup;
        {
            ProfScope ps(ctx, logr == 12 ? "lde_copy_probe_a<12>" : logr == 11 ? "lde_copy_probe_a<11>" : "lde_copy_probe_a<10>", (4.0 * n + 4.0 * N) * batch);
            const dim3 grid(a.n_tiles, batch);
            if (logr == 10) lde_a_probe_kernel<10><<<grid, 256, 0, ctx->stream>>>(a);
            if (logr == 11) lde_a_probe_kernel<11><<<grid, 512, 0, ctx->stream>>>(a);
            if (logr == 12) lde_a_probe_kernel<12><<<grid, 1024, 0, ctx->stream>>>(a);
        }
        a.n_tiles = 1u << (logN - SMI_LDE_LOGB - SMI_LDE_BLINES_LOG);
        {
            ProfScope ps(ctx, "lde_copy_probe_b", 8.0 * N * batch);
            lde_b_probe_kernel<<<dim3(((a.dbg >> 8) & 255u) == 3 ? a.n_tiles / 2 : a.n_tiles, batch), 1024, 0, ctx->stream>>>(a);
        }
        HIP_TRY(ctx, hipGetLastError());
        return SMI_OK;
    }
    {
        a.n_tiles = 256u << log_blowup;
        const dim3 grid(a.n_tiles, batch);
        ProfScope ps(ctx, logr == 12 ? "lde_a_kernel<12>" : logr == 11 ? "lde_a_kernel<11>" : "lde_a_kernel<10>", (4.0 * n + 4.0 * N) * batch);
#define LA(LR)                                                                                     \
    if (logr == LR) {                                                                              \
        if (wide) lde_a_kernel<LR, 8><<<grid, 1 << (LR - 2), 0, ctx->stream>>>(a);                 \
        else lde_a_kernel<LR, 4><<<grid, 1 << (LR - 2), 0, ctx->stream>>>(a);                      \
    }
        LA(10) LA(11) LA(12)
#undef LA
        HIP_TRY(ctx, hipGetLastError());
    }
    {
        a.n_tiles = 1u << (logN - SMI_LDE_LOGB - SMI_LDE_BLINES_LOG);
        const dim3 grid(a.n_tiles, batch);
        ProfScope ps(ctx, "lde_b_kernel", 8.0 * N * batch);
        if (wide) lde_b_kernel<8><<<grid, 1024, 0, ctx->stream>>>(a);
        else lde_b_kernel<4><<<grid, 1024, 0, ctx->stream>>>(a);
        HIP_TRY(ctx, hipGetLastError());
    }
    return SMI_OK;
}

int dev_ntt(smi_ctx *ctx, const uint32_t *d_in, uint32_t *d_out, uint32_t log_n, size_t n_in, uint32_t batch,
            size_t in_stride, size_t out_stride, int inverse, uint64_t offset, uint64_t post_scale) {
    const uint32_t p = ctx->fs.F.p;
    if (log_n > ctx->fs.K)
        return smi_fail(ctx, p == 998244353u ? SMI_ERR_ROOT_TOO_LARGE : SMI_ERR_UNSUPPORTED_PRIME,
                        "transform size exceeds the two-adicity of the modulus");
    const uint64_t n = 1ull << log_n;
    if (!batch) return SMI_OK;
    if (n_in > n || (inverse && n_in != n)) return smi_fail(ctx, SMI_ERR_BAD_ARG, "n_in out of range");
    if (offset >= p || post_scale >= p) return smi_fail(ctx, SMI_ERR_NON_CANONICAL, "offset/post_scale must be < p");
    if (offset == 0) return smi_fail(ctx, SMI_ERR_NO_INVERSE, "offset must be invertible");
    if (batch > 65535) return smi_fail(ctx, SMI_ERR_BAD_ARG, "batch too large");

    if (n_in == 0) {
        for (uint32_t c = 0; c < batch; c++) HIP_TRY(ctx, hipMemsetAsync(d_out + (size_t)c * out_stride, 0, n * 4, ctx->stream));
        return SMI_OK;
    }
    ScaleScope pin__(ctx);
    NttRequest rq;
    memset(&rq, 0, sizeof rq);
    rq.in = d_in; rq.out = d_out; rq.L = log_n; rq.n_in = (uint32_t)n_in; rq.batch = batch;
    rq.in_stride = in_stride; rq.out_stride = out_stride; rq.F = ctx->fs.F;
    rq.T = ctx_tables(ctx, inverse);
    if (!inverse) {
        rq.pre_scale = offset != 1;
        rq.q_plain = (uint32_t)offset;
        if (rq.pre_scale) SMI_TRY(ctx_scale_tables(ctx, 1, (uint32_t)offset, log_n, &rq.S));
    } else {
        rq.post_scale = true;
        const uint32_t ninv = h_inv(ctx, (uint32_t)(n % p));
        const uint32_t q = h_mul(ctx, (uint32_t)post_scale, h_inv(ctx, (uint32_t)offset));
        rq.q_plain = q;
        SMI_TRY(ctx_scale_tables(ctx, ninv, q, log_n, &rq.S));
    }
    rq.defer_tw = ctx->ntt_defer_tw;
    rq.last_direct = ctx->ntt_last_direct;
    if (ntt_make_plan(log_n, batch).np > 0) SMI_TRY(ctx_scratch(ctx, (size_t)batch << log_n, &rq.scratch));
    HipLauncher ln{ctx};
    if (!ntt_run(ln, rq)) return smi_fail(ctx, SMI_ERR_BAD_ARG, "ntt: multi-pass plan without its inter-pass buffer");
    if (ln.err != hipSuccess) return smi_hip_fail(ctx, ln.err, "ntt kernel launch");
    return SMI_OK;
}

static int shard_request(smi_ctx *ctx, uint32_t log_n, int inverse, uint64_t offset, NttRequest *rq) {
    const uint32_t p = ctx->fs.F.p;
    if (log_n > ctx->fs.K)
        return smi_fail(ctx, p == 998244353u ? SMI_ERR_ROOT_TOO_LARGE : SMI_ERR_UNSUPPORTED_PRIME, "transform size exceeds the two-adicity of the modulus");
    if (offset >= p) return smi_fail(ctx, SMI_ERR_NON_CANONICAL, "offset must be < p");
    if (offset == 0) return smi_fail(ctx, SMI_ERR_NO_INVERSE, "offset must be invertible");
    if (inverse && offset != 1) return smi_fail(ctx, SMI_ERR_BAD_ARG, "sharded inverse transform: offset must be 1");
    memset(rq, 0, sizeof *rq);
    rq->L = log_n; rq->n_in = (uint32_t)(1ull << log_n); rq->batch = 1; rq->F = ctx->fs.F;
    rq->T = ctx_tables(ctx, inverse);
    if (!inverse) {
        rq->pre_scale = offset != 1;
        rq->q_plain = (uint32_t)offset;
        if (rq->pre_scale) SMI_TRY(ctx_scale_tables(ctx, 1, (uint32_t)offset, log_n, &rq->S));
    } else {
        rq->post_scale = true;
        rq->q_plain = 1;
        SMI_TRY(ctx_scale_tables(ctx, h_inv(ctx, (uint32_t)((1ull << log_n) % p)), 1, log_n, &rq->S));
    }
    return SMI_OK;
}
int dev_ntt_shard_first(smi_ctx *ctx, uint32_t *d_strip, uint32_t log_n, uint32_t log_g, uint32_t rank, int inverse, uint64_t offset) {
    ScaleScope pin__(ctx);
    NttRequest rq;
    SMI_TRY(shard_request(ctx, log_n, inverse, offset, &rq));
    rq.in = d_strip; rq.out = d_strip;
    HipLauncher ln{ctx};
    if (!ntt_run_shard_first(ln, rq, log_g, rank)) return smi_fail(ctx, SMI_ERR_BAD_ARG, "sharded transform: size too small for this many ranks");
    if (ln.err != hipSuccess) return smi_hip_fail(ctx, ln.err, "ntt kernel launch");
    return SMI_OK;
}
int dev_ntt_shard_rest(smi_ctx *ctx, uint32_t *d_rows, uint32_t *d_out, uint32_t log_n, uint32_t log_g, int inverse) {
    ScaleScope pin__(ctx);
    NttRequest rq;
    SMI_TRY(shard_request(ctx, log_n, inverse, 1, &rq));
    rq.scratch = d_rows; rq.out = d_out;
    rq.last_direct = ctx->ntt_last_direct;
    HipLauncher ln{ctx};
    if (!ntt_run_shard_rest(ln, rq, log_g)) return smi_fail(ctx, SMI_ERR_BAD_ARG, "sharded transform: size too small for this many ranks");
    if (ln.err != hipSuccess) return smi_hip_fail(ctx, ln.err, "ntt kernel launch");
    return SMI_OK;
}
```

### stark_rs_amd/csrc/ntt_core.h

```cpp
#pragma once
#include "field.h"

#if defined(SMI_EMU_CHECKS) && !defined(__HIP_DEVICE_COMPILE__)
#include <assert.h>
#define SMI_BOUND_CHECK(x, m, p) assert((m) <= 8 && (uint64_t)(x) < (uint64_t)((m) ? (m) : 1) * (p) && ((m) || (x) == 0))
#else
#define SMI_BOUND_CHECK(x, m, p) ((void)0)
#endif

#define SMI_TILE_LOG 12
#define SMI_TILE (1u << SMI_TILE_LOG)
#define SMI_NTT_THREADS 256
#define SMI_TW_LOG 12

struct alignas(8) Tw2 {
    uint32_t w, q;
};

struct NttTables {
    const Tw2 *tw10;
    const uint32_t *lo;
    const uint32_t *hi;
    uint32_t K, h;
};
struct ScaleTables {
    const uint32_t *lo, *hi;
    uint32_t h;
};
enum { NTT_FIRST = 1, NTT_PRE_SCALE = 2, NTT_POST_SCALE = 4, NTT_TW_SKIP = 8, NTT_TW_IN = 16, NTT_LAST_DIRECT = 32 };

struct PassArgs {
    const uint32_t *in;
    uint32_t *out;
    uint64_t in_stride, out_stride;
    Fp F;
    NttTables T;
    ScaleTables S;
    uint32_t L;
    uint32_t Sp;
    uint32_t n_in;
    uint32_t flags;
    uint32_t d0_log;
    uint32_t n_mid;
    uint32_t mid_log[2];
    uint32_t n_tiles;
    uint32_t batch;
    uint32_t pre_ratio_m;
    uint32_t post_ratio_m;
    uint32_t post_bi_ratio_m;
    uint32_t zlog;
    uint32_t shard_log, b_off;
    uint32_t prev_logr;
};

enum { SMI_COLS_PER_WG = 4, SMI_COLS_MIN_WGS = 1024 };

template <int LOGR> struct Steps;
template <> struct Steps<6>  { enum { n = 2, s0 = 4, s1 = 2, s2 = 0 }; };
template <> struct Steps<7>  { enum { n = 2, s0 = 4, s1 = 3, s2 = 0 }; };
template <> struct Steps<8>  { enum { n = 2, s0 = 4, s1 = 4, s2 = 0 }; };
template <> struct Steps<9>  { enum { n = 3, s0 = 4, s1 = 3, s2 = 2 }; };
template <> struct Steps<10> { enum { n = 3, s0 = 4, s1 = 3, s2 = 3 }; };
template <> struct Steps<11> { enum { n = 3, s0 = 4, s1 = 4, s2 = 3 }; };

template <int S> SMI_HD constexpr uint32_t brev(uint32_t x) {
    uint32_t r = 0;
    for (int i = 0; i < S; i++) r |= ((x >> i) & 1u) << (S - 1 - i);
    return r;
}

SMI_HD uint32_t xcd_tile(uint32_t b, uint32_t n_tiles) {
    if (n_tiles % 8u) return b;
    return (b & 7u) * (n_tiles >> 3) + (b >> 3);
}

SMI_HD uint32_t two_level(const uint32_t *lo, const uint32_t *hi, uint32_t h, uint32_t e, const Fp &F) {
    return mont_mul(lo[e & ((1u << h) - 1u)], hi[e >> h], F);
}

#ifndef SMI_NTT_NT
#define SMI_NTT_NT 0
#endif
SMI_HD uint32_t ld32(const uint32_t *base, uint32_t idx) {
    const uint32_t *p = (const uint32_t *)((const char *)base + (size_t)(uint32_t)(idx << 2));
#if defined(__HIP_DEVICE_COMPILE__) && SMI_NTT_NT
    return __builtin_nontemporal_load(p);
#else
    return *p;
#endif
}
SMI_HD void st32(uint32_t *base, uint32_t idx, uint32_t v) {
    uint32_t *p = (uint32_t *)((char *)base + (size_t)(uint32_t)(idx << 2));
#if defined(SMI_NTT_DBG_NOSTORE)
    if (v != 0xFFFFFFFFu) return;
#endif
#if defined(__HIP_DEVICE_COMPILE__) && SMI_NTT_NT
    __builtin_nontemporal_store(v, p);
#else
    *p = v;
#endif
}
SMI_HD Tw2 ld_tw(const Tw2 *base, uint32_t idx) { return *(const Tw2 *)((const char *)base + (size_t)(uint32_t)(idx << 3)); }

SMI_HD uint32_t shoup_mul(uint32_t a, const Tw2 &c, uint32_t p) {
    return a * c.w - umulhi32(a, c.q) * p;
}
SMI_HD uint32_t lz_canon(uint32_t a, uint32_t p) { return umin32(a, a - p); }

SMI_HD void lz_fold_m(uint32_t &x, int &m, uint32_t p) {
    if (m > 4) { x = umin32(x, x - 4u * p); m = 4; }
    else if (m > 2) { x = umin32(x, x - 2u * p); m = 2; }
}
SMI_HD void lz_fold_to2(uint32_t &x, int &m, uint32_t p) {
    lz_fold_m(x, m, p);
    lz_fold_m(x, m, p);
}
SMI_HD uint32_t lz_canon_m(uint32_t x, int m, uint32_t p) {
    lz_fold_to2(x, m, p);
    return m > 1 ? umin32(x, x - p) : x;
}

template <int S, int CAP, int Z = 0>
SMI_HD void dft_regs(uint32_t (&x)[1 << S], int (&m)[1 << S], const Tw2 *cw, int croot_shift, const Fp &F) {
    const uint32_t p = F.p;
#pragma unroll
    for (int s = 0; s < S; s++) {
        const int half = (1 << S) >> (s + 1);
#pragma unroll
        for (int i = 0; i < (1 << S); i++) {
            if (i & half) continue;
            const int j = i | half;
            const int e = (i & (half - 1)) << s;
            if (s < Z) {
                x[j] = e ? shoup_mul(x[i], cw[e << croot_shift], p) : x[i];
                m[j] = e ? 2 : m[i];
                continue;
            }
#pragma unroll
            for (int t = 0; t < 3; t++)
                if (m[i] + m[j] > CAP) {
                    if (m[i] >= m[j]) lz_fold_m(x[i], m[i], p);
                    else lz_fold_m(x[j], m[j], p);
                }
            const uint32_t u = x[i], v = x[j];
            const int ms = m[i] + m[j];
            SMI_BOUND_CHECK(u, m[i], p);
            SMI_BOUND_CHECK(v, m[j], p);
            x[i] = u + v;
            const uint32_t d = u - v + (uint32_t)m[j] * p;
            m[i] = ms;
            if (e) { x[j] = shoup_mul(d, cw[e << croot_shift], p); m[j] = 2; }
            else { x[j] = d; m[j] = ms; }
        }
    }
}

enum { PASS_FIRST = 0, PASS_MID = 1, PASS_LAST = 2 };
template <int LOGR, int LOGW, int KIND, int CAP> struct NttPass {
    static constexpr bool FIRST = KIND == PASS_FIRST, MID = KIND == PASS_MID, LAST = KIND == PASS_LAST;
    enum { TILE_LOG = LOGR + LOGW, TILE = 1 << TILE_LOG, NT = TILE / 16, R = 1 << LOGR, W = 1 << LOGW, WP = W + 1, V = 16 };
    typedef Steps<LOGR> St;
    enum { SL = St::n == 2 ? St::s1 : St::s2, RL = 1 << SL };

    struct TileId {
        uint64_t in_base, out_base;
        uint32_t b0;
    };

    static SMI_HD TileId tile_id(const PassArgs &a, uint32_t block) {
        TileId t;
        const uint32_t tix = xcd_tile(block, a.n_tiles);
        if (!LAST) {
            const uint32_t ablog = a.L - a.Sp - LOGR - a.shard_log;
            const uint32_t tpa = 1u << (ablog - LOGW);
            const uint32_t sub = tix / tpa;
            t.b0 = (tix % tpa) << LOGW;
            t.in_base = ((uint64_t)sub << (a.L - a.Sp - a.shard_log)) + t.b0;
            t.out_base = t.in_base;
        } else {
            const uint32_t g0 = 1u << (a.d0_log - LOGW);
            const uint32_t a_rest = tix / g0;
            const uint32_t k0_0 = (tix % g0) << LOGW;
            const uint32_t arest_log = a.Sp - a.d0_log;
            uint32_t rev = 0, shift_in = arest_log, shift_out = 0;
            for (uint32_t d = 0; d < a.n_mid; d++) {
                shift_in -= a.mid_log[d];
                rev |= ((a_rest >> shift_in) & ((1u << a.mid_log[d]) - 1u)) << shift_out;
                shift_out += a.mid_log[d];
            }
            t.b0 = k0_0;
            t.in_base = (((uint64_t)k0_0 << arest_log) + a_rest) << LOGR;
            t.out_base = ((uint64_t)rev << a.d0_log) + k0_0;
        }
        return t;
    }

    static SMI_HD void load_tw(const PassArgs &a, Tw2 *tw, uint32_t tid) {
#pragma unroll
        for (int i = 0; i < (R + NT - 1) / NT; i++) {
            uint32_t j = tid + i * NT;
            if (j < (uint32_t)R) tw[j] = a.T.tw10[j << (SMI_TW_LOG - LOGR)];
        }
    }

    template <int Z, bool TWIN = true> static SMI_HD void load_regs(const PassArgs &a, const TileId &t, uint32_t batch, uint32_t (&v)[V], uint32_t tid) {
        const uint32_t blog = a.L - a.Sp - LOGR, ablog = blog - a.shard_log;
        const uint32_t w = tid & (W - 1), j0 = tid >> LOGW;
        const uint32_t o0 = (j0 << ablog) + w;
        if constexpr (FIRST) {
            const uint32_t *col = a.in + (uint64_t)batch * a.in_stride;
            const uint32_t n0 = a.b_off + t.b0 + (j0 << blog) + w;
#pragma unroll
            for (int i = 0; i < V; i++) {
                if (i >= (V >> Z)) { v[i] = 0u; continue; }
                const uint32_t g = n0 + ((uint32_t)(i * (NT >> LOGW)) << blog);
                const uint32_t ga = t.b0 + o0 + ((uint32_t)(i * (NT >> LOGW)) << ablog);
                const uint32_t x = ld32(col, g < a.n_in ? ga : 0u);
                v[i] = g < a.n_in ? x : 0u;
            }
            if (a.flags & NTT_PRE_SCALE) {
                uint32_t sc = two_level(a.S.lo, a.S.hi, a.S.h, n0, a.F);
                const uint32_t rq = a.pre_ratio_m * a.F.pinv;
#pragma unroll
                for (int i = 0; i < (V >> Z); i++) {
                    v[i] = mont_mul(v[i], sc, a.F);
                    sc = mont_mul_c(sc, a.pre_ratio_m, rq, a.F);
                }
            }
        } else {
            const uint32_t *in = a.in + (uint64_t)batch * a.in_stride + t.in_base;
#pragma unroll
            for (int i = 0; i < V; i++) v[i] = ld32(in, o0 + ((uint32_t)(i * (NT >> LOGW)) << ablog));
            if (TWIN && (a.flags & NTT_TW_IN)) {
                const uint32_t sub = (uint32_t)(t.in_base >> (a.L - a.Sp)), k = sub & ((1u << a.prev_logr) - 1u);
                const uint32_t sh = a.T.K - (a.L - a.Sp + a.prev_logr);
                uint32_t cur = two_level(a.T.lo, a.T.hi, a.T.h, (k * ((j0 << blog) + t.b0 + w)) << sh, a.F);
                const uint32_t ratio = two_level(a.T.lo, a.T.hi, a.T.h, (k * ((uint32_t)(NT >> LOGW) << blog)) << sh, a.F);
                const uint32_t rq = ratio * a.F.pinv;
#pragma unroll
                for (int i = 0; i < V; i++) {
                    v[i] = mont_mul(v[i], cur, a.F);
                    if (i + 1 < V) cur = mont_mul_c(cur, ratio, rq, a.F);
                }
            }
        }
    }

    template <int Z> static SMI_HD void step0_regs(const PassArgs &a, uint32_t (&x)[V], uint32_t *tile, const Tw2 *tw, uint32_t tid) {
        enum { SUB = LOGR - 4 };
        const uint32_t w = tid & (W - 1), pos = tid >> LOGW;
        int m[16];
#pragma unroll
        for (int i = 0; i < 16; i++) m[i] = i < (V >> Z) ? 1 : 0;
        dft_regs<4, CAP, Z>(x, m, tw, LOGR - 4, a.F);
#pragma unroll
        for (int kk = 0; kk < 16; kk++) {
            uint32_t v = x[brev<4>(kk)];
            int mv = m[brev<4>(kk)];
            if (kk) v = shoup_mul(v, tw[(pos * kk) & (R - 1)], a.F.p);
            else lz_fold_to2(v, mv, a.F.p);
            tile[(pos + ((uint32_t)kk << SUB)) * WP + w] = v;
        }
    }

    static SMI_HD void load_rows(const PassArgs &a, const TileId &t, uint32_t batch, uint32_t (&v)[V], uint32_t tid) {
        const uint32_t *in = a.in + (uint64_t)batch * a.in_stride + t.in_base;
        const uint32_t arest_log = a.Sp - a.d0_log;
#pragma unroll
        for (int i = 0; i < V; i++) {
            const uint32_t idx = tid + i * NT;
            const uint32_t j = idx & (R - 1), l = idx >> LOGR;
            v[i] = ld32(in, (l << (arest_log + LOGR)) + j);
        }
    }
    static SMI_HD void rows_to_lds(const uint32_t (&v)[V], uint32_t *tile, uint32_t tid) {
#pragma unroll
        for (int i = 0; i < V; i++) {
            const uint32_t idx = tid + i * NT;
            tile[(idx & (R - 1)) * WP + (idx >> LOGR)] = v[i];
        }
    }

    static SMI_HD void direct_map(uint32_t tid, uint32_t &pos, uint32_t &line) {
        enum { SUB = LOGR - 4, ROT = SUB >= 5 ? 0 : SUB % LOGW };
        pos = tid & ((1u << SUB) - 1u);
        const uint32_t lsel = tid >> SUB;
        if constexpr (ROT != 0) line = ((lsel << ROT) | (lsel >> (LOGW - ROT))) & (W - 1);
        else line = lsel;
    }
    static SMI_HD void load_rows_direct(const PassArgs &a, const TileId &t, uint32_t batch, uint32_t (&v)[V], uint32_t tid) {
        enum { SUB = LOGR - 4 };
        const uint32_t *in = a.in + (uint64_t)batch * a.in_stride + t.in_base;
        const uint32_t arest_log = a.Sp - a.d0_log;
        uint32_t pos, line;
        direct_map(tid, pos, line);
        const uint32_t o0 = (line << (arest_log + LOGR)) + pos;
#pragma unroll
        for (int i = 0; i < V; i++) v[i] = ld32(in, o0 + ((uint32_t)i << SUB));
    }
    static SMI_HD void step0_rows(const PassArgs &a, uint32_t (&x)[V], uint32_t *tile, const Tw2 *tw, uint32_t tid) {
        enum { SUB = LOGR - 4 };
        uint32_t pos, line;
        direct_map(tid, pos, line);
        int m[16];
#pragma unroll
        for (int i = 0; i < 16; i++) m[i] = 1;
        dft_regs<4, CAP>(x, m, tw, LOGR - 4, a.F);
#pragma unroll
        for (int kk = 0; kk < 16; kk++) {
            uint32_t v = x[brev<4>(kk)];
            int mv = m[brev<4>(kk)];
            if (kk) v = shoup_mul(v, tw[(pos * kk) & (R - 1)], a.F.p);
            else lz_fold_to2(v, mv, a.F.p);
            tile[(pos + ((uint32_t)kk << SUB)) * WP + line] = v;
        }
    }

    template <int S, int MLOG, int MIN> static SMI_HD void step(const PassArgs &a, uint32_t *tile, const Tw2 *tw, uint32_t tid) {
        enum { r = 1 << S, SUB = MLOG - S, NB = (TILE / r) / NT };
#pragma unroll
        for (int bi = 0; bi < NB; bi++) {
            const uint32_t u = tid + bi * NT;
            const uint32_t w = u & (W - 1), ub = u >> LOGW;
            const uint32_t blk = ub >> SUB, pos = ub & ((1u << SUB) - 1u);
            const uint32_t base = (blk << MLOG) + pos;
            uint32_t x[r];
#pragma unroll
            for (int q = 0; q < r; q++) x[q] = tile[(base + ((uint32_t)q << SUB)) * WP + w];
            int m[r];
#pragma unroll
            for (int q = 0; q < r; q++) m[q] = MIN;
            dft_regs<S, CAP>(x, m, tw, LOGR - S, a.F);
#pragma unroll
            for (int kk = 0; kk < r; kk++) {
                uint32_t v = x[brev<S>(kk)];
                int mv = m[brev<S>(kk)];
                if (kk) v = shoup_mul(v, tw[((pos * kk) << (LOGR - MLOG)) & (R - 1)], a.F.p);
                else lz_fold_to2(v, mv, a.F.p);
                tile[(base + ((uint32_t)kk << SUB)) * WP + w] = v;
            }
        }
    }
    static SMI_HD void step0_lds(const PassArgs &a, uint32_t *tile, const Tw2 *tw, uint32_t tid) { step<4, LOGR, 1>(a, tile, tw, tid); }
    static SMI_HD void step_mid(const PassArgs &a, uint32_t *tile, const Tw2 *tw, uint32_t tid) {
        if constexpr (St::n == 3) step<St::s1, LOGR - St::s0, 2>(a, tile, tw, tid);
    }

    static SMI_HD uint32_t blk_to_k(uint32_t blk) {
        if (St::n == 2) return blk;
        const uint32_t k0 = blk >> St::s1, k1 = blk & ((1u << St::s1) - 1u);
        return k0 | (k1 << St::s0);
    }

    static SMI_HD void last_step_store(const PassArgs &a, const TileId &t, uint32_t batch, const uint32_t *tile, const Tw2 *tw,
                                       uint32_t tid) {
        enum { NB = (TILE / RL) / NT, KSTEP_LOG = LOGR - SL };
        uint32_t *out = a.out + (uint64_t)batch * a.out_stride + t.out_base;
        const uint32_t mlog = a.L - a.Sp, p = a.F.p;
        uint32_t base_run = 0, gs = 0, gq = 0, gbi = 0, gbq = 0;
        uint32_t sc_run = 0, rq = 0, rbq = 0;
        if (!LAST && !(a.flags & NTT_TW_SKIP)) {
            const uint32_t b = a.b_off + t.b0 + (tid & (W - 1)), sh = a.T.K - mlog;
            base_run = two_level(a.T.lo, a.T.hi, a.T.h, (b * blk_to_k(tid >> LOGW)) << sh, a.F);
            gs = two_level(a.T.lo, a.T.hi, a.T.h, (b << KSTEP_LOG) << sh, a.F);
            gq = gs * a.F.pinv;
            if (NB > 1) {
                gbi = two_level(a.T.lo, a.T.hi, a.T.h, (b << SL) << sh, a.F);
                gbq = gbi * a.F.pinv;
            }
        }
        if (LAST && (a.flags & NTT_POST_SCALE)) {
            sc_run = two_level(a.S.lo, a.S.hi, a.S.h, (uint32_t)t.out_base + (blk_to_k(tid >> LOGW) << a.Sp) + (tid & (W - 1)), a.F);
            rq = a.post_ratio_m * a.F.pinv;
            rbq = a.post_bi_ratio_m * a.F.pinv;
        }
#pragma unroll
        for (int bi = 0; bi < NB; bi++) {
            const uint32_t u = tid + bi * NT;
            const uint32_t w = u & (W - 1), blk = u >> LOGW;
            uint32_t x[RL];
#pragma unroll
            for (int q = 0; q < RL; q++) x[q] = tile[(blk * RL + q) * WP + w];
            int m[RL];
#pragma unroll
            for (int q = 0; q < RL; q++) m[q] = 2;
            dft_regs<SL, CAP>(x, m, tw, LOGR - SL, a.F);
            const uint32_t kbase = blk_to_k(blk);
            if constexpr (!LAST) {
                const uint32_t blog = mlog - LOGR - a.shard_log;
                const uint32_t o0 = (kbase << blog) + w;
                {
                    if (a.flags & NTT_TW_SKIP) {
#pragma unroll
                        for (int kk = 0; kk < RL; kk++) {
                            SMI_BOUND_CHECK(x[brev<SL>(kk)], m[brev<SL>(kk)], p);
                            st32(out, o0 + ((uint32_t)kk << (KSTEP_LOG + blog)), x[brev<SL>(kk)]);
                        }
                        continue;
                    }
                    uint32_t cur = base_run;
                    if (bi + 1 < NB) base_run = mont_mul_c(base_run, gbi, gbq, a.F);
#pragma unroll
                    for (int kk = 0; kk < RL; kk++) {
                        st32(out, o0 + ((uint32_t)kk << (KSTEP_LOG + blog)), mont_mul(x[brev<SL>(kk)], cur, a.F));
                        if (kk + 1 < RL) cur = mont_mul_c(cur, gs, gq, a.F);
                    }
                }
            } else {
                const uint32_t o0 = (kbase << a.Sp) + w;
                if (a.flags & NTT_POST_SCALE) {
                    uint32_t sc = sc_run;
                    if (bi + 1 < NB) sc_run = mont_mul_c(sc_run, a.post_bi_ratio_m, rbq, a.F);
#pragma unroll
                    for (int kk = 0; kk < RL; kk++) {
                        st32(out, o0 + ((uint32_t)kk << (KSTEP_LOG + a.Sp)), mont_mul(x[brev<SL>(kk)], sc, a.F));
                        if (kk + 1 < RL) sc = mont_mul_c(sc, a.post_ratio_m, rq, a.F);
                    }
                } else {
#pragma unroll
                    for (int kk = 0; kk < RL; kk++) st32(out, o0 + ((uint32_t)kk << (KSTEP_LOG + a.Sp)), lz_canon_m(x[brev<SL>(kk)], m[brev<SL>(kk)], p));
                }
            }
        }
    }

    static SMI_HD bool has_out_mul(const PassArgs &a) { return LAST ? (a.flags & NTT_POST_SCALE) != 0 : !(a.flags & NTT_TW_SKIP); }
    enum { COLS_PER_WG = SMI_COLS_PER_WG, COLS_MIN_WGS = SMI_COLS_MIN_WGS };
    static SMI_HD uint32_t col_groups(const PassArgs &a) { return (a.batch + COLS_PER_WG - 1) / COLS_PER_WG; }
    static SMI_HD bool share_cols(const PassArgs &a, uint32_t min_wgs = COLS_MIN_WGS) {
        return !FIRST && a.batch > 1 && has_out_mul(a) && (uint64_t)a.n_tiles * col_groups(a) >= min_wgs;
    }
    template <bool MQ = true>
    static SMI_HD void out_mul(const PassArgs &a, const TileId &t, uint32_t tid, uint32_t (&mw)[V], uint32_t (&mq)[MQ ? V : 1]) {
        enum { NB = (TILE / RL) / NT, KSTEP_LOG = LOGR - SL };
        const uint32_t w = tid & (W - 1), kb0 = blk_to_k(tid >> LOGW);
        uint32_t run, step, step_bi = 0;
        if (!LAST) {
            const uint32_t b = a.b_off + t.b0 + w, sh = a.T.K - (a.L - a.Sp);
            run = two_level(a.T.lo, a.T.hi, a.T.h, (b * kb0) << sh, a.F);
            step = two_level(a.T.lo, a.T.hi, a.T.h, (b << KSTEP_LOG) << sh, a.F);
            if (NB > 1) step_bi = two_level(a.T.lo, a.T.hi, a.T.h, (b << SL) << sh, a.F);
        } else {
            run = two_level(a.S.lo, a.S.hi, a.S.h, (uint32_t)t.out_base + (kb0 << a.Sp) + w, a.F);
            step = a.post_ratio_m;
            step_bi = a.post_bi_ratio_m;
        }
        const uint32_t sq = step * a.F.pinv, bq = step_bi * a.F.pinv;
#pragma unroll
        for (int bi = 0; bi < NB; bi++) {
            uint32_t cur = run;
            if (bi + 1 < NB) run = mont_mul_c(run, step_bi, bq, a.F);
#pragma unroll
            for (int kk = 0; kk < RL; kk++) {
                mw[bi * RL + kk] = cur;
                if constexpr (MQ) mq[bi * RL + kk] = cur * a.F.pinv;
                if (kk + 1 < RL) cur = mont_mul_c(cur, step, sq, a.F);
            }
        }
    }
    static SMI_HD void in_mul(const PassArgs &a, const TileId &t, uint32_t tid, uint32_t (&iw)[V]) {
        const uint32_t blog = a.L - a.Sp - LOGR;
        const uint32_t w = tid & (W - 1), j0 = tid >> LOGW;
        const uint32_t sub = (uint32_t)(t.in_base >> (a.L - a.Sp)), k = sub & ((1u << a.prev_logr) - 1u);
        const uint32_t sh = a.T.K - (a.L - a.Sp + a.prev_logr);
        uint32_t cur = two_level(a.T.lo, a.T.hi, a.T.h, (k * ((j0 << blog) + t.b0 + w)) << sh, a.F);
        const uint32_t ratio = two_level(a.T.lo, a.T.hi, a.T.h, (k * ((uint32_t)(NT >> LOGW) << blog)) << sh, a.F);
        const uint32_t rq = ratio * a.F.pinv;
#pragma unroll
        for (int i = 0; i < V; i++) {
            iw[i] = cur;
            if (i + 1 < V) cur = mont_mul_c(cur, ratio, rq, a.F);
        }
    }
    template <bool MQ = true>
    static SMI_HD void last_step_store_mul(const PassArgs &a, const TileId &t, uint32_t batch, const uint32_t *tile, const Tw2 *tw,
                                           uint32_t tid, const uint32_t (&mw)[V], const uint32_t (&mq)[MQ ? V : 1]) {
        enum { NB = (TILE / RL) / NT, KSTEP_LOG = LOGR - SL };
        uint32_t *out = a.out + (uint64_t)batch * a.out_stride + t.out_base;
        const uint32_t olog = LAST ? a.Sp : a.L - a.Sp - LOGR - a.shard_log;
#pragma unroll
        for (int bi = 0; bi < NB; bi++) {
            const uint32_t u = tid + bi * NT;
            const uint32_t w = u & (W - 1), blk = u >> LOGW;
            uint32_t x[RL];
#pragma unroll
            for (int q = 0; q < RL; q++) x[q] = tile[(blk * RL + q) * WP + w];
            int m[RL];
#pragma unroll
            for (int q = 0; q < RL; q++) m[q] = 2;
            dft_regs<SL, CAP>(x, m, tw, LOGR - SL, a.F);
            const uint32_t o0 = (blk_to_k(blk) << olog) + w;
#pragma unroll
            for (int kk = 0; kk < RL; kk++)
                if constexpr (MQ) st32(out, o0 + ((uint32_t)kk << (KSTEP_LOG + olog)), mont_mul_c(x[brev<SL>(kk)], mw[bi * RL + kk], mq[bi * RL + kk], a.F));
                else st32(out, o0 + ((uint32_t)kk << (KSTEP_LOG + olog)), mont_mul(x[brev<SL>(kk)], mw[bi * RL + kk], a.F));
        }
    }
};

struct SmallArgs {
    const uint32_t *in;
    uint32_t *out;
    uint64_t in_stride, out_stride;
    Fp F;
    NttTables T;
    ScaleTables S;
    uint32_t L, n_in, flags;
};
struct NttSmall {
    static SMI_HD uint32_t at(uint32_t i) { return i + (i >> 6); }
    static SMI_HD void load_tw(const SmallArgs &a, Tw2 *twm, uint32_t tid) {
        const uint32_t half_n = (1u << a.L) >> 1;
        for (uint32_t j = tid; j < half_n; j += SMI_NTT_THREADS) twm[j] = a.T.tw10[j << (SMI_TW_LOG - a.L)];
    }
    static SMI_HD void load(const SmallArgs &a, uint32_t batch, uint32_t *buf, uint32_t tid) {
        const uint32_t n = 1u << a.L;
        const uint32_t *in = a.in + (uint64_t)batch * a.in_stride;
        for (uint32_t g = tid; g < n; g += SMI_NTT_THREADS) {
            uint32_t v = g < a.n_in ? in[g] : 0u;
            if ((a.flags & NTT_PRE_SCALE) && v) v = mont_mul(v, two_level(a.S.lo, a.S.hi, a.S.h, g, a.F), a.F);
            buf[at(g)] = v;
        }
    }
    static SMI_HD uint32_t mulw(uint32_t x, const Tw2 &w, uint32_t p) { return lz_canon(shoup_mul(x, w, p), p); }
    static SMI_HD void stage4(const SmallArgs &a, uint32_t s, uint32_t *buf, const Tw2 *twm, uint32_t tid) {
        const uint32_t n = 1u << a.L, qlog = a.L - s - 2, q = 1u << qlog, p = a.F.p;
        for (uint32_t u = tid; u < n / 4; u += SMI_NTT_THREADS) {
            const uint32_t blk = u >> qlog, pos = u & (q - 1);
            const uint32_t i = (blk << (qlog + 2)) + pos;
            const uint32_t x0 = buf[at(i)], x1 = buf[at(i + q)], x2 = buf[at(i + 2 * q)], x3 = buf[at(i + 3 * q)];
            const uint32_t a0 = fp_add(x0, x2, p), a1 = fp_add(x1, x3, p);
            const uint32_t c0 = mulw(fp_sub(x0, x2, p), twm[pos << s], p);
            const uint32_t c1 = mulw(fp_sub(x1, x3, p), twm[(pos + q) << s], p);
            const Tw2 w = twm[pos << (s + 1)];
            buf[at(i)] = fp_add(a0, a1, p);
            buf[at(i + q)] = mulw(fp_sub(a0, a1, p), w, p);
            buf[at(i + 2 * q)] = fp_add(c0, c1, p);
            buf[at(i + 3 * q)] = mulw(fp_sub(c0, c1, p), w, p);
        }
    }
    static SMI_HD void stage(const SmallArgs &a, uint32_t s, uint32_t *buf, const Tw2 *twm, uint32_t tid) {
        const uint32_t n = 1u << a.L, hlog = a.L - s - 1, half = 1u << hlog;
        for (uint32_t u = tid; u < n / 2; u += SMI_NTT_THREADS) {
            const uint32_t blk = u >> hlog, pos = u & (half - 1);
            const uint32_t i = (blk << (hlog + 1)) + pos, j = i + half;
            const uint32_t x = buf[at(i)], y = buf[at(j)];
            buf[at(i)] = fp_add(x, y, a.F.p);
            buf[at(j)] = mulw(fp_sub(x, y, a.F.p), twm[pos << s], a.F.p);
        }
    }
    static SMI_HD void store(const SmallArgs &a, uint32_t batch, const uint32_t *buf, uint32_t tid) {
        const uint32_t n = 1u << a.L;
        uint32_t *out = a.out + (uint64_t)batch * a.out_stride;
        for (uint32_t k = tid; k < n; k += SMI_NTT_THREADS) {
            uint32_t v = buf[at(a.L ? bitrev32(k) >> (32u - a.L) : 0u)];
            if (a.flags & NTT_POST_SCALE) v = mont_mul(v, two_level(a.S.lo, a.S.hi, a.S.h, k, a.F), a.F);
            out[k] = v;
        }
    }
};
```

### stark_rs_amd/csrc/tables.h

```cpp
#pragma once
#include "ntt_host.h"

struct GeomSpec {
    uint32_t c_m, q_m;
    uint64_t stride;
    uint32_t count;
    uint32_t pair;
};

struct FieldSetup {
    Fp F;
    uint32_t g;
    uint32_t K;
    uint32_t wmax[2];
};

inline bool is_prime_u32(uint32_t n) {
    if (n < 2) return false;
    for (uint32_t q : {2u, 3u, 5u, 7u, 11u, 13u}) {
        if (n == q) return true;
        if (n % q == 0) return false;
    }
    uint32_t d = n - 1, r = 0;
    while (!(d & 1)) { d >>= 1; r++; }
    for (uint32_t a : {2u, 7u, 61u}) {
        uint32_t x = host_powmod(a % n, d, n);
        if (x == 1 || x == n - 1 || a % n == 0) continue;
        bool witness = true;
        for (uint32_t i = 1; i < r && witness; i++) {
            x = host_mulmod(x, x, n);
            if (x == n - 1) witness = false;
        }
        if (witness) return false;
    }
    return true;
}

inline bool field_setup(uint64_t p64, uint64_t g64, FieldSetup *fs) {
    if (p64 < 3 || p64 >= (1ull << 30) || (p64 & 1) == 0 || g64 == 0 || g64 >= p64) return false;
    const uint32_t p = (uint32_t)p64, g = (uint32_t)g64;
    if (!is_prime_u32(p)) return false;
    uint32_t two_adicity = 0;
    while (((p - 1) >> two_adicity) % 2 == 0) two_adicity++;
    if (two_adicity < SMI_TILE_LOG) return false;
    fs->F = fp_make(p);
    fs->g = g;
    fs->K = two_adicity > 27 ? 27 : two_adicity;
    const uint32_t w = host_powmod(g, (p - 1) >> fs->K, p);
    if (host_powmod(w, 1ull << (fs->K - 1), p) != p - 1) return false;
    fs->wmax[0] = w;
    fs->wmax[1] = host_powmod(w, p - 2, p);
    return true;
}

inline uint32_t ntt_table_h(uint32_t K) { return (K + 1) / 2; }

inline void ntt_table_specs(const FieldSetup &fs, int inverse, GeomSpec specs[3]) {
    const Fp &F = fs.F;
    const uint32_t w_m = (uint32_t)(((uint64_t)fs.wmax[inverse ? 1 : 0] << 32) % F.p);
    const uint32_t h = ntt_table_h(fs.K);
    specs[0] = GeomSpec{F.r1, w_m, 1ull << (fs.K - SMI_TW_LOG), 1u << SMI_TW_LOG, 1};
    specs[1] = GeomSpec{F.r1, w_m, 1, 1u << h, 0};
    specs[2] = GeomSpec{F.r1, w_m, 1ull << h, 1u << (fs.K - h), 0};
}

inline uint32_t scale_table_h(uint32_t L) { return (L + 1) / 2; }
inline void scale_table_specs(const Fp &F, uint32_t c_plain, uint32_t q_plain, uint32_t L, GeomSpec specs[2]) {
    const uint32_t c_m = (uint32_t)(((uint64_t)c_plain << 32) % F.p), q_m = (uint32_t)(((uint64_t)q_plain << 32) % F.p);
    const uint32_t h = scale_table_h(L);
    specs[0] = GeomSpec{F.r1, q_m, 1, 1u << h, 0};
    specs[1] = GeomSpec{c_m, q_m, 1ull << h, 1u << (L - h), 0};
}

SMI_HD Tw2 tw2_from_mont(uint32_t v_m, const Fp &F) {
    const uint32_t w = from_mont(v_m, F);
    return Tw2{w, (uint32_t)(((uint64_t)w << 32) / F.p)};
}
```

Baseline: 229.6 billion field-elements/s.

## Pass 16-point twiddles as kernel args and double-buffer LDS tiles in twin column pass

Precomputes the eight 16th-root twiddles on the host and passes them in the table struct, so register DFT stages read kernel arguments instead of the shared-memory twiddle array. For the twiddle-in mid column pass with two radix stages, it also allocates two LDS tiles and alternates between them per column. This lets the next column's global load overlap the current column's store and removes one barrier per column. The cost is doubled shared memory for that kernel, which may reduce occupancy, and a larger kernel-argument struct.

```diff
diff --git a/stark_rs_amd/csrc/api.hip b/stark_rs_amd/csrc/api.hip
--- a/stark_rs_amd/csrc/api.hip
+++ b/stark_rs_amd/csrc/api.hip
@@ -77,6 +77,7 @@
         for (int dir = 0; dir < 2 && rc == SMI_OK; dir++) {
             GeomSpec sp[3];
             ntt_table_specs(ctx->fs, dir, sp);
+            ntt_w16_fill(ctx->fs, dir, ctx->w16[dir]);
             for (int k = 0; k < 3 && rc == SMI_OK; k++) {
                 if (hipMalloc((void **)&ctx->d_tab[dir][k], ((size_t)sp[k].count * 4) << sp[k].pair) != hipSuccess) { rc = SMI_ERR_OOM; break; }
                 rc = launch_geom_table(ctx, sp[k], ctx->d_tab[dir][k]);
@@ -266,7 +267,7 @@
 }
 NttTables ctx_tables(const smi_ctx *ctx, int inverse) {
     const int d = inverse ? 1 : 0;
-    return NttTables{(const Tw2 *)ctx->d_tab[d][0], ctx->d_tab[d][1], ctx->d_tab[d][2], ctx->fs.K, ntt_table_h(ctx->fs.K)};
+    return ntt_tables_make(ctx->fs, ctx->w16[d], ctx->d_tab[d][0], ctx->d_tab[d][1], ctx->d_tab[d][2]);
 }
 int ctx_root_table(smi_ctx *ctx, uint32_t log_m, const Tw2 **out) {
     if (log_m > 17 || log_m > ctx->fs.K) return smi_fail(ctx, SMI_ERR_BAD_ARG, "root table too large");
diff --git a/stark_rs_amd/csrc/emu.cpp b/stark_rs_amd/csrc/emu.cpp
--- a/stark_rs_amd/csrc/emu.cpp
+++ b/stark_rs_amd/csrc/emu.cpp
@@ -1,3 +1,4 @@
+#include <algorithm>
 #include <array>
 #include <vector>
 
@@ -22,15 +23,18 @@
     typedef NttPass<LOGR, LOGW, KIND, CAP> NP;
     constexpr bool LAST = KIND == PASS_LAST;
     const uint32_t NT = NP::NT;
-    std::vector<uint32_t> tile(NP::R * NP::WP);
+    const bool twin = KIND == PASS_MID && (a.flags & NTT_TW_IN);
+    const bool two_tiles = twin && NP::template cols_two_tiles<true>();
+    const size_t tile_words = NP::R * NP::WP;
+    std::vector<uint32_t> tiles((two_tiles ? 2 : 1) * tile_words);
     std::vector<Tw2> tw(NP::R);
     std::vector<std::array<uint32_t, 16>> mw(NT), mq(NT), iw(NT), regs(NT);
-    const bool twin = KIND == PASS_MID && (a.flags & NTT_TW_IN);
     auto r16 = [](std::array<uint32_t, 16> &x) -> uint32_t(&)[16] { return reinterpret_cast<uint32_t(&)[16]>(x); };
     for (uint32_t blk = 0; blk < a.n_tiles; blk++) {
         typename NP::TileId t = NP::tile_id(a, blk);
         for (uint32_t tid = 0; tid < NT; tid++) NP::load_tw(a, tw.data(), tid);
         for (uint32_t b = 0; b < a.batch; b++) {
+            uint32_t *const tile = tiles.data() + (two_tiles ? (b & 1u) * tile_words : 0);
             if (b % NP::COLS_PER_WG == 0)
                 for (uint32_t tid = 0; tid < NT; tid++) {
                     NP::out_mul(a, t, tid, r16(mw[tid]), r16(mq[tid]));
@@ -41,25 +45,28 @@
                     NP::template load_regs<0, false>(a, t, b, r16(regs[tid]), tid);
                     for (int i = 0; i < 16; i++) regs[tid][i] = mont_mul(regs[tid][i], iw[tid][i], a.F);
                 }
-                for (uint32_t tid = 0; tid < NT; tid++) NP::template step0_regs<0>(a, r16(regs[tid]), tile.data(), tw.data(), tid);
+                for (uint32_t tid = 0; tid < NT; tid++) NP::template step0_regs<0>(a, r16(regs[tid]), tile, tw.data(), tid);
             } else if (!LAST) {
 #define ZCASE(Z)                                                                                                 \
     case Z:                                                                                                      \
         for (uint32_t tid = 0; tid < NT; tid++) NP::template load_regs<Z>(a, t, b, r16(regs[tid]), tid);         \
-        for (uint32_t tid = 0; tid < NT; tid++) NP::template step0_regs<Z>(a, r16(regs[tid]), tile.data(), tw.data(), tid); \
+        for (uint32_t tid = 0; tid < NT; tid++) NP::template step0_regs<Z>(a, r16(regs[tid]), tile, tw.data(), tid); \
         break;
                 switch (a.zlog) { ZCASE(2) ZCASE(3) ZCASE(4) default: ZCASE(0) }
 #undef ZCASE
             } else if (a.flags & NTT_LAST_DIRECT) {
                 for (uint32_t tid = 0; tid < NT; tid++) NP::load_rows_direct(a, t, b, r16(regs[tid]), tid);
-                for (uint32_t tid = 0; tid < NT; tid++) NP::step0_rows(a, r16(regs[tid]), tile.data(), tw.data(), tid);
+                for (uint32_t tid = 0; tid < NT; tid++) NP::step0_rows(a, r16(regs[tid]), tile, tw.data(), tid);
             } else {
                 for (uint32_t tid = 0; tid < NT; tid++) NP::load_rows(a, t, b, r16(regs[tid]), tid);
-                for (uint32_t tid = 0; tid < NT; tid++) NP::rows_to_lds(r16(regs[tid]), tile.data(), tid);
-                for (uint32_t tid = 0; tid < NT; tid++) NP::step0_lds(a, tile.data(), tw.data(), tid);
+                for (uint32_t tid = 0; tid < NT; tid++) NP::rows_to_lds(r16(regs[tid]), tile, tid);
+                for (uint32_t tid = 0; tid < NT; tid++) NP::step0_lds(a, tile, tw.data(), tid);
             }
-            for (uint32_t tid = 0; tid < NT; tid++) NP::step_mid(a, tile.data(), tw.data(), tid);
-            for (uint32_t tid = 0; tid < NT; tid++) NP::last_step_store_mul(a, t, b, tile.data(), tw.data(), tid, r16(mw[tid]), r16(mq[tid]));
+            for (uint32_t tid = 0; tid < NT; tid++) NP::step_mid(a, tile, tw.data(), tid);
+            for (uint32_t tid = 0; tid < NT; tid++) NP::last_step_store_mul(a, t, b, tile, tid, r16(mw[tid]), r16(mq[tid]));
+#ifdef SMI_EMU_CHECKS
+            if (two_tiles) std::fill(tile, tile + tile_words, 1u);
+#endif
         }
     }
 }
@@ -99,7 +106,7 @@
                 for (uint32_t tid = 0; tid < NT; tid++) NP::step0_lds(a, tile.data(), tw.data(), tid);
             }
             for (uint32_t tid = 0; tid < NT; tid++) NP::step_mid(a, tile.data(), tw.data(), tid);
-            for (uint32_t tid = 0; tid < NT; tid++) NP::last_step_store(a, t, b, tile.data(), tw.data(), tid);
+            for (uint32_t tid = 0; tid < NT; tid++) NP::last_step_store(a, t, b, tile.data(), tid);
         }
 }
 
@@ -154,7 +161,9 @@
     std::vector<uint32_t> tw10 = fill(sp[0], F), lo = fill(sp[1], F), hi = fill(sp[2], F);
     NttRequest rq;
     memset(&rq, 0, sizeof rq);
-    rq.T = NttTables{(const Tw2 *)tw10.data(), lo.data(), hi.data(), fs.K, ntt_table_h(fs.K)};
+    Tw2 w16[8];
+    ntt_w16_fill(fs, inverse, w16);
+    rq.T = ntt_tables_make(fs, w16, tw10.data(), lo.data(), hi.data());
     std::vector<uint32_t> slo, shi;
     const uint32_t pp = F.p;
     if (!inverse) {
@@ -182,6 +191,25 @@
     rq.last_direct = g_emu_last_direct;
     EmuLauncher ln;
     return ntt_run(ln, rq) ? 0 : -1;
+}
+
+extern "C" int emu_ntt_w16(uint64_t p, uint64_t g, int inverse, uint32_t *w16_out, uint32_t *ref) {
+    FieldSetup fs;
+    if (!field_setup(p, g, &fs)) return -1;
+    GeomSpec sp[3];
+    ntt_table_specs(fs, inverse, sp);
+    const std::vector<uint32_t> tw10 = fill(sp[0], fs.F), lo = fill(sp[1], fs.F), hi = fill(sp[2], fs.F);
+    Tw2 w16[8];
+    ntt_w16_fill(fs, inverse, w16);
+    const NttTables T = ntt_tables_make(fs, w16, tw10.data(), lo.data(), hi.data());
+    for (uint32_t e = 0; e < 8; e++) {
+        w16_out[2 * e] = T.w16[e].w;
+        w16_out[2 * e + 1] = T.w16[e].q;
+        const Tw2 r = T.tw10[e << (SMI_TW_LOG - 4)];
+        ref[2 * e] = r.w;
+        ref[2 * e + 1] = r.q;
+    }
+    return 0;
 }
 
 namespace {
@@ -197,7 +225,9 @@
     ntt_table_specs(fs, inverse, sp);
     t.tw10 = fill(sp[0], F); t.lo = fill(sp[1], F); t.hi = fill(sp[2], F);
     memset(&t.rq, 0, sizeof t.rq);
-    t.rq.T = NttTables{(const Tw2 *)t.tw10.data(), t.lo.data(), t.hi.data(), fs.K, ntt_table_h(fs.K)};
+    Tw2 w16[8];
+    ntt_w16_fill(fs, inverse, w16);
+    t.rq.T = ntt_tables_make(fs, w16, t.tw10.data(), t.lo.data(), t.hi.data());
     t.rq.L = L; t.rq.n_in = 1u << L; t.rq.batch = 1; t.rq.F = F;
     if (!inverse) {
         t.rq.pre_scale = offset % F.p != 1;
@@ -239,9 +269,9 @@
             std::vector<std::array<uint32_t, 16>> regs(A::NT);
             for (uint32_t tid = 0; tid < A::NT; tid++) A::load_tw(a, tw.data(), tid);
             for (uint32_t tid = 0; tid < A::NT; tid++) A::load_regs(a, t, b, reinterpret_cast<uint32_t(&)[16]>(regs[tid]), tid);
-            for (uint32_t tid = 0; tid < A::NT; tid++) A::step0(a, reinterpret_cast<uint32_t(&)[16]>(regs[tid]), tile.data(), tw.data(), tid);
+            for (uint32_t tid = 0; tid < A::NT; tid++) A::step0(a, reinterpret_cast<uint32_t(&)[16]>(regs[tid]), tile.data(), tid);
             for (uint32_t tid = 0; tid < A::NT; tid++) A::step_mid(a, tile.data(), tw.data(), tid);
-            for (uint32_t tid = 0; tid < A::NT; tid++) A::last_step_store(a, t, b, tile.data(), tw.data(), tid);
+            for (uint32_t tid = 0; tid < A::NT; tid++) A::last_step_store(a, t, b, tile.data(), tid);
         }
 }
 template <int CAP> void emu_lde_b(const LdeArgs &a) {
@@ -259,7 +289,7 @@
             }
             for (uint32_t tid = 0; tid < B::NT; tid++) B::step0(a, t, tile.data(), tw.data(), tid);
             for (uint32_t tid = 0; tid < B::NT; tid++) B::step_mid(a, tile.data(), tw.data(), tid);
-            for (uint32_t tid = 0; tid < B::NT; tid++) B::last_step_store(a, t, b, tile.data(), tw.data(), tid);
+            for (uint32_t tid = 0; tid < B::NT; tid++) B::last_step_store(a, t, b, tile.data(), tid);
         }
 }
 static int g_emu_lde_geo = -1, g_emu_lde_lay = -1;
@@ -278,7 +308,9 @@
     LdeArgs a;
     memset(&a, 0, sizeof a);
     a.coef = coef; a.mid = mid.data(); a.coef_t = coef_t.data(); a.ctab = (const Tw2 *)ctab.data(); a.out = out; a.coef_stride = 1ull << L; a.out_stride = 1ull << (L + beta);
-    a.F = F; a.T = NttTables{(const Tw2 *)tw10.data(), lo.data(), hi.data(), fs.K, ntt_table_h(fs.K)};
+    Tw2 w16[8];
+    ntt_w16_fill(fs, 0, w16);
+    a.F = F; a.T = ntt_tables_make(fs, w16, tw10.data(), lo.data(), hi.data());
     a.L = L; a.beta = beta; a.batch = batch;
     a.geo_rq = g_emu_lde_geo >= 0 && (uint32_t)g_emu_lde_geo <= beta ? (uint32_t)g_emu_lde_geo : lde_default_geo_rq(beta);
     a.lay_kq = g_emu_lde_lay >= (int)(SMI_LDE_BLINES_LOG - a.geo_rq) && g_emu_lde_lay <= 4 ? (uint32_t)g_emu_lde_lay : SMI_LDE_BLINES_LOG - a.geo_rq;
diff --git a/stark_rs_amd/csrc/internal.h b/stark_rs_amd/csrc/internal.h
--- a/stark_rs_amd/csrc/internal.h
+++ b/stark_rs_amd/csrc/internal.h
@@ -31,6 +31,7 @@
     bool own_stream = false;
     FieldSetup fs;
     uint32_t *d_tab[2][3] = {{nullptr, nullptr, nullptr}, {nullptr, nullptr, nullptr}};
+    Tw2 w16[2][8] = {};
     std::vector<ScaleEntry> scale_cache;
     uint64_t scale_epoch = 1;
     int scale_depth = 0;
diff --git a/stark_rs_amd/csrc/lde_core.h b/stark_rs_amd/csrc/lde_core.h
--- a/stark_rs_amd/csrc/lde_core.h
+++ b/stark_rs_amd/csrc/lde_core.h
@@ -85,7 +85,7 @@
             for (int i = 0; i < V; i++) v[i] = shoup_mul(v[i], ld_tw(a.ctab, (e0 + (uint32_t)i * es) & mask), a.F.p);
         }
     }
-    static SMI_HD void step0(const LdeArgs &a, uint32_t (&x)[V], uint32_t *tile, const Tw2 *tw, uint32_t tid) {
+    static SMI_HD void step0(const LdeArgs &a, uint32_t (&x)[V], uint32_t *tile, uint32_t tid) {
         const uint32_t w = tid & 3u, pos = tid >> 2, pos_sw = lde_swz(pos);
         int m[16];
 #pragma unroll
@@ -93,7 +93,7 @@
         Tw2 t0[16];
 #pragma unroll
         for (int kk = 1; kk < 16; kk++) t0[kk] = ld_tw(a.T.tw10, ((pos * kk) & (R - 1)) << (SMI_TW_LOG - LOGR));
-        dft_regs<4, CAP>(x, m, tw, LOGR - 8, a.F);
+        dft_regs<4, CAP>(x, m, a.T.w16, 0, a.F);
 #pragma unroll
         for (int kk = 0; kk < 16; kk++) {
             uint32_t v = x[brev<4>(kk)];
@@ -118,7 +118,7 @@
                 x[q] = tile[((base_sw ^ lde_swz((uint32_t)q << SUB)) << 2) + w];
                 m[q] = 2;
             }
-            dft_regs<S, CAP>(x, m, tw, MLOG - S, a.F);
+            dft_regs<S, CAP>(x, m, a.T.w16, 4 - S, a.F);
 #pragma unroll
             for (int kk = 0; kk < r; kk++) {
                 uint32_t v = x[brev<S>(kk)];
@@ -129,8 +129,7 @@
             }
         }
     }
-    static SMI_HD void last_step_store(const LdeArgs &a, const TileId &t, uint32_t batch, const uint32_t *tile, const Tw2 *tw,
-                                       uint32_t tid) {
+    static SMI_HD void last_step_store(const LdeArgs &a, const TileId &t, uint32_t batch, const uint32_t *tile, uint32_t tid) {
         enum { S1 = St::s1, SL = St::s2 };
         uint32_t *mid = a.mid + ((uint64_t)batch << (a.L + a.beta));
 #pragma unroll
@@ -145,7 +144,7 @@
                 x[q] = tile[((blk_sw ^ lde_swz((uint32_t)q)) << 2) + w];
                 m[q] = 2;
             }
-            dft_regs<SL, CAP>(x, m, tw, LOGR - 4 - SL, a.F);
+            dft_regs<SL, CAP>(x, m, a.T.w16, 4 - SL, a.F);
             const uint32_t k1b = d0 | (d1 << 4);
             const uint32_t kq = a.lay_kq;
             const uint32_t o0 = ((((k1b >> kq) << a.beta) + t.r) << (10 + kq)) + (t.jt << (kq + 2)) + ((k1b & ((1u << kq) - 1u)) << 2) + w;
@@ -247,7 +246,7 @@
             m[q] = 1;
             if (q + 1 < 16) cur = mont_mul_c(cur, ratio, rq, a.F);
         }
-        dft_regs<4, CAP>(x, m, tw, SMI_LDE_LOGB - 4, a.F);
+        dft_regs<4, CAP>(x, m, a.T.w16, 0, a.F);
 #pragma unroll
         for (int kk = 0; kk < 16; kk++) {
             uint32_t v = x[brev<4>(kk)];
@@ -260,10 +259,10 @@
     static SMI_HD void step_mid(const LdeArgs &a, uint32_t *tile, const Tw2 *tw, uint32_t tid) {
         PassArgs pa;
         pa.F = a.F;
+        pa.T = a.T;
         NP::step_mid(pa, tile, tw, tid);
     }
-    static SMI_HD void last_step_store(const LdeArgs &a, const TileId &t, uint32_t batch, const uint32_t *tile, const Tw2 *tw,
-                                       uint32_t tid) {
+    static SMI_HD void last_step_store(const LdeArgs &a, const TileId &t, uint32_t batch, const uint32_t *tile, uint32_t tid) {
         const Geo g = geo(a);
         uint32_t *out = a.out + (uint64_t)batch * a.out_stride;
         const uint32_t logRA = a.L - SMI_LDE_LOGB, ksh = a.beta + logRA;
@@ -279,7 +278,7 @@
                 x[q] = tile[(blk * RL + q) * WP + l];
                 m[q] = 2;
             }
-            dft_regs<SL, CAP>(x, m, tw, SMI_LDE_LOGB - SL, a.F);
+            dft_regs<SL, CAP>(x, m, a.T.w16, 4 - SL, a.F);
             const uint32_t k0b = NP::blk_to_k(blk);
             const uint32_t lineoff = ((l & ((1u << g.kq_bits) - 1u)) << a.beta) + (l >> g.kq_bits);
             const uint32_t o0 = (k0b << ksh) + base + lineoff;
diff --git a/stark_rs_amd/csrc/ntt.hip b/stark_rs_amd/csrc/ntt.hip
--- a/stark_rs_amd/csrc/ntt.hip
+++ b/stark_rs_amd/csrc/ntt.hip
@@ -39,7 +39,7 @@
         NP::step_mid(a, tile, tw, tid);
         __syncthreads();
     }
-    NP::last_step_store(a, t, batch, tile, tw, tid);
+    NP::last_step_store(a, t, batch, tile, tid);
 }
 
 #ifndef SMI_COLS_WAVES
@@ -57,7 +57,8 @@
 template <int LOGR, int LOGW, int KIND, int CAP, bool TWIN = false>
 __global__ __launch_bounds__(1 << (LOGR + LOGW - 4), TWIN ? SMI_COLS_TWIN_WAVES : SMI_COLS_WAVES(LOGR + LOGW, LOGR)) void ntt_pass_cols_kernel(const PassArgs a) {
     typedef NttPass<LOGR, LOGW, KIND, CAP> NP;
-    __shared__ uint32_t tile[NP::R * NP::WP];
+    constexpr bool TWO_TILES = SMI_COLS_PREFETCH && NP::template cols_two_tiles<TWIN>();
+    __shared__ uint32_t tile[(TWO_TILES ? 2 : 1) * NP::R * NP::WP];
     __shared__ Tw2 tw[NP::R];
     const uint32_t tid0 = threadIdx.x;
     const typename NP::TileId t = NP::tile_id(a, blockIdx.x);
@@ -76,6 +77,21 @@
             NP::template load_regs<0, !TWIN>(a, t, col, v, tid);
         };
         load(col0);
+        if constexpr (TWO_TILES) {
+            __syncthreads();
+            for (uint32_t batch = col0; batch < col1; batch++) {
+                uint32_t tid = tid0;
+                asm volatile("" : "+v"(tid));
+                uint32_t *tb = tile + (batch & 1u) * (uint32_t)(NP::R * NP::WP);
+#pragma unroll
+                for (int i = 0; i < NP::V; i++) v[i] = mont_mul(v[i], iw[i], a.F);
+                NP::template step0_regs<0>(a, v, tb, tw, tid);
+                if (batch + 1 < col1) load(batch + 1);
+                __syncthreads();
+                NP::template last_step_store_mul<MQ>(a, t, batch, tb, tid, mw, mq);
+            }
+            return;
+        }
         for (uint32_t batch = col0; batch < col1; batch++) {
             uint32_t tid = tid0;
             asm volatile("" : "+v"(tid));
@@ -91,7 +107,7 @@
                 NP::step_mid(a, tile, tw, tid);
                 __syncthreads();
             }
-            NP::template last_step_store_mul<MQ>(a, t, batch, tile, tw, tid, mw, mq);
+            NP::template last_step_store_mul<MQ>(a, t, batch, tile, tid, mw, mq);
         }
         return;
     }
@@ -124,7 +140,7 @@
             NP::step_mid(a, tile, tw, tid);
             __syncthreads();
         }
-        NP::template last_step_store_mul<MQ>(a, t, batch, tile, tw, tid, mw, mq);
+        NP::template last_step_store_mul<MQ>(a, t, batch, tile, tid, mw, mq);
     }
 }
 
@@ -187,11 +203,11 @@
     uint32_t v[A::V];
     A::load_regs(a, t, batch, v, tid);
     __syncthreads();
-    A::step0(a, v, tile, tw, tid);
+    A::step0(a, v, tile, tid);
     __syncthreads();
     A::step_mid(a, tile, tw, tid);
     __syncthreads();
-    A::last_step_store(a, t, batch, tile, tw, tid);
+    A::last_step_store(a, t, batch, tile, tid);
 }
 template <int CAP>
 __global__ __launch_bounds__(1024) void lde_b_kernel(const LdeArgs a) {
@@ -209,7 +225,7 @@
     __syncthreads();
     B::step_mid(a, tile, tw, tid);
     __syncthreads();
-    B::last_step_store(a, t, batch, tile, tw, tid);
+    B::last_step_store(a, t, batch, tile, tid);
 }
 
 template <int LOGR> __global__ __launch_bounds__(1 << (LOGR - 2)) void lde_a_probe_kernel(const LdeArgs a) {
diff --git a/stark_rs_amd/csrc/ntt_core.h b/stark_rs_amd/csrc/ntt_core.h
--- a/stark_rs_amd/csrc/ntt_core.h
+++ b/stark_rs_amd/csrc/ntt_core.h
@@ -22,6 +22,7 @@
     const uint32_t *lo;
     const uint32_t *hi;
     uint32_t K, h;
+    Tw2 w16[8];
 };
 struct ScaleTables {
     const uint32_t *lo, *hi;
@@ -121,7 +122,8 @@
 }
 
 template <int S, int CAP, int Z = 0>
-SMI_HD void dft_regs(uint32_t (&x)[1 << S], int (&m)[1 << S], const Tw2 *cw, int croot_shift, const Fp &F) {
+SMI_HD void dft_regs(uint32_t (&x)[1 << S], int (&m)[1 << S], const Tw2 *cw, int cshift, const Fp &F) {
+    static_assert(S >= 1 && S <= 4, "register butterflies of 2..16 points");
     const uint32_t p = F.p;
 #pragma unroll
     for (int s = 0; s < S; s++) {
@@ -132,7 +134,7 @@
             const int j = i | half;
             const int e = (i & (half - 1)) << s;
             if (s < Z) {
-                x[j] = e ? shoup_mul(x[i], cw[e << croot_shift], p) : x[i];
+                x[j] = e ? shoup_mul(x[i], cw[e << cshift], p) : x[i];
                 m[j] = e ? 2 : m[i];
                 continue;
             }
@@ -149,7 +151,7 @@
             x[i] = u + v;
             const uint32_t d = u - v + (uint32_t)m[j] * p;
             m[i] = ms;
-            if (e) { x[j] = shoup_mul(d, cw[e << croot_shift], p); m[j] = 2; }
+            if (e) { x[j] = shoup_mul(d, cw[e << cshift], p); m[j] = 2; }
             else { x[j] = d; m[j] = ms; }
         }
     }
@@ -252,7 +254,8 @@
         int m[16];
 #pragma unroll
         for (int i = 0; i < 16; i++) m[i] = i < (V >> Z) ? 1 : 0;
-        dft_regs<4, CAP, Z>(x, m, tw, LOGR - 4, a.F);
+        if constexpr (FIRST) dft_regs<4, CAP, Z>(x, m, tw, LOGR - 4, a.F);
+        else dft_regs<4, CAP, Z>(x, m, a.T.w16, 0, a.F);
 #pragma unroll
         for (int kk = 0; kk < 16; kk++) {
             uint32_t v = x[brev<4>(kk)];
@@ -305,7 +308,7 @@
         int m[16];
 #pragma unroll
         for (int i = 0; i < 16; i++) m[i] = 1;
-        dft_regs<4, CAP>(x, m, tw, LOGR - 4, a.F);
+        dft_regs<4, CAP>(x, m, a.T.w16, 0, a.F);
 #pragma unroll
         for (int kk = 0; kk < 16; kk++) {
             uint32_t v = x[brev<4>(kk)];
@@ -330,7 +333,7 @@
             int m[r];
 #pragma unroll
             for (int q = 0; q < r; q++) m[q] = MIN;
-            dft_regs<S, CAP>(x, m, tw, LOGR - S, a.F);
+            dft_regs<S, CAP>(x, m, a.T.w16, 4 - S, a.F);
 #pragma unroll
             for (int kk = 0; kk < r; kk++) {
                 uint32_t v = x[brev<S>(kk)];
@@ -352,8 +355,7 @@
         return k0 | (k1 << St::s0);
     }
 
-    static SMI_HD void last_step_store(const PassArgs &a, const TileId &t, uint32_t batch, const uint32_t *tile, const Tw2 *tw,
-                                       uint32_t tid) {
+    static SMI_HD void last_step_store(const PassArgs &a, const TileId &t, uint32_t batch, const uint32_t *tile, uint32_t tid) {
         enum { NB = (TILE / RL) / NT, KSTEP_LOG = LOGR - SL };
         uint32_t *out = a.out + (uint64_t)batch * a.out_stride + t.out_base;
         const uint32_t mlog = a.L - a.Sp, p = a.F.p;
@@ -384,7 +386,7 @@
             int m[RL];
 #pragma unroll
             for (int q = 0; q < RL; q++) m[q] = 2;
-            dft_regs<SL, CAP>(x, m, tw, LOGR - SL, a.F);
+            dft_regs<SL, CAP>(x, m, a.T.w16, 4 - SL, a.F);
             const uint32_t kbase = blk_to_k(blk);
             if constexpr (!LAST) {
                 const uint32_t blog = mlog - LOGR - a.shard_log;
@@ -430,6 +432,8 @@
     static SMI_HD bool share_cols(const PassArgs &a, uint32_t min_wgs = COLS_MIN_WGS) {
         return !FIRST && a.batch > 1 && has_out_mul(a) && (uint64_t)a.n_tiles * col_groups(a) >= min_wgs;
     }
+    template <bool TWIN> static constexpr bool cols_two_tiles() { return TWIN && MID && LOGW == 5 && St::n == 2 && TILE_LOG <= 13; }
+
     template <bool MQ = true>
     static SMI_HD void out_mul(const PassArgs &a, const TileId &t, uint32_t tid, uint32_t (&mw)[V], uint32_t (&mq)[MQ ? V : 1]) {
         enum { NB = (TILE / RL) / NT, KSTEP_LOG = LOGR - SL };
@@ -473,8 +477,8 @@
         }
     }
     template <bool MQ = true>
-    static SMI_HD void last_step_store_mul(const PassArgs &a, const TileId &t, uint32_t batch, const uint32_t *tile, const Tw2 *tw,
-                                           uint32_t tid, const uint32_t (&mw)[V], const uint32_t (&mq)[MQ ? V : 1]) {
+    static SMI_HD void last_step_store_mul(const PassArgs &a, const TileId &t, uint32_t batch, const uint32_t *tile, uint32_t tid,
+                                           const uint32_t (&mw)[V], const uint32_t (&mq)[MQ ? V : 1]) {
         enum { NB = (TILE / RL) / NT, KSTEP_LOG = LOGR - SL };
         uint32_t *out = a.out + (uint64_t)batch * a.out_stride + t.out_base;
         const uint32_t olog = LAST ? a.Sp : a.L - a.Sp - LOGR - a.shard_log;
@@ -488,7 +492,7 @@
             int m[RL];
 #pragma unroll
             for (int q = 0; q < RL; q++) m[q] = 2;
-            dft_regs<SL, CAP>(x, m, tw, LOGR - SL, a.F);
+            dft_regs<SL, CAP>(x, m, a.T.w16, 4 - SL, a.F);
             const uint32_t o0 = (blk_to_k(blk) << olog) + w;
 #pragma unroll
             for (int kk = 0; kk < RL; kk++)
diff --git a/stark_rs_amd/csrc/tables.h b/stark_rs_amd/csrc/tables.h
--- a/stark_rs_amd/csrc/tables.h
+++ b/stark_rs_amd/csrc/tables.h
@@ -64,6 +64,21 @@
     specs[2] = GeomSpec{F.r1, w_m, 1ull << h, 1u << (fs.K - h), 0};
 }
 
+inline void ntt_w16_fill(const FieldSetup &fs, int inverse, Tw2 (&w16)[8]) {
+    const uint32_t p = fs.F.p, w = host_powmod(fs.wmax[inverse ? 1 : 0], 1ull << (fs.K - 4), p);
+    uint32_t cur = 1;
+    for (int e = 0; e < 8; e++) {
+        w16[e] = Tw2{cur, (uint32_t)(((uint64_t)cur << 32) / p)};
+        cur = host_mulmod(cur, w, p);
+    }
+}
+inline NttTables ntt_tables_make(const FieldSetup &fs, const Tw2 (&w16)[8], const uint32_t *tw10, const uint32_t *lo, const uint32_t *hi) {
+    NttTables T;
+    T.tw10 = (const Tw2 *)tw10; T.lo = lo; T.hi = hi; T.K = fs.K; T.h = ntt_table_h(fs.K);
+    for (int e = 0; e < 8; e++) T.w16[e] = w16[e];
+    return T;
+}
+
 inline uint32_t scale_table_h(uint32_t L) { return (L + 1) / 2; }
 inline void scale_table_specs(const Fp &F, uint32_t c_plain, uint32_t q_plain, uint32_t L, GeomSpec specs[2]) {
     const uint32_t c_m = (uint32_t)(((uint64_t)c_plain << 32) % F.p), q_m = (uint32_t)(((uint64_t)q_plain << 32) % F.p);
```

Result: slower. 219.4 billion field-elements/s (-4.5%).
